# SinOncology/BreakID

Measured on AMD Instinct MI355X. Metric: M reads/s clustered+split-scanned, higher is better.
Workload: dtype int32/u8 (+f64 sd replay)

## Files before the change

breakid_amd/capi.py:

```python
from __future__ import annotations

import ctypes as C
import math
import os
import subprocess

import numpy as np

from . import abi

_HERE = os.path.dirname(os.path.abspath(__file__))
LIB_PATH = os.path.join(_HERE, "libbreakid_hip.so")
_LIB = None


class BreakIDError(RuntimeError):
    def __init__(self, code, msg):
        super().__init__("libbreakid_hip error %d: %s" % (code, msg))
        self.code = code


def build(verbose=False):
    cmd = ["make", "-C", os.path.join(_HERE, "csrc"), "-j8"]
    r = subprocess.run(cmd, capture_output=not verbose, text=True)
    if r.returncode != 0:
        raise RuntimeError("building libbreakid_hip.so failed:\n" + (r.stdout or "")[-4000:] + (r.stderr or "")[-4000:])


EXPORTS = ["bk_init", "bk_prepare_process", "bk_free", "bk_last_error", "bk_set_stream", "bk_sync", "bk_get_stream", "bk_upload_records", "bk_isize_stats",
           "bk_discordant_pairs", "bk_mask_and_cluster", "bk_split_evidence", "bk_cluster_summary",
           "bk_split_breakpoints", "bk_run", "bk_fetch", "bk_timing", "bk_timing_enable", "bk_timing_touched", "bk_group_stats", "bk_qname_hash", "bk_qname_check",
           "bk_bam_open", "bk_bam_header", "bk_bam_decode", "bk_bam_close", "bk_bam_decode_device", "bk_bam_decode_device_part", "bk_bam_decode_device_ctx", "bk_bam_dev_free", "bk_feed_release_caches", "bk_debug_bgzf_inflate", "bk_debug_std_sort", "bk_debug_ahc", "bk_debug_points", "bk_debug_cigar", "bk_debug_vote", "bk_debug_region", "bk_shard_begin", "bk_shard_get_stats", "bk_shard_set_stats",
           "bk_shard_sd_local", "bk_shard_sd_finish", "bk_shard_buffer", "bk_shard_set_buffer", "bk_shard_group_sizes",
           "bk_shard_own_groups", "bk_shard_route_candidates", "bk_shard_group_keys", "bk_shard_route_pairs", "bk_shard_group_pairs", "bk_shard_bp_cov", "bk_shard_bp_vote", "bk_shard_bp_vote_slice", "bk_shard_bp_set_voted", "bk_shard_bp_depth", "bk_shard_bp_finish"]


def lib():
    global _LIB
    if _LIB is None:
        if not os.path.exists(LIB_PATH):
            raise BreakIDError(abi.BK_ERR_NO_DEVICE, "libbreakid_hip.so is not built (run __graft_entry__.build()); "
                                                     "there is no CPU fallback")
        try:
            import torch
        except Exception:
            pass
        L = C.CDLL(LIB_PATH)
        vp, u64p, dp = C.c_void_p, C.POINTER(C.c_uint64), C.POINTER(C.c_double)
        L.bk_init.argtypes = [C.c_int, vp, C.POINTER(C.c_char_p), C.c_int, C.POINTER(vp)]
        L.bk_free.argtypes = [vp]
        L.bk_last_error.restype = C.c_char_p
        L.bk_last_error.argtypes = [vp]
        L.bk_set_stream.argtypes = [vp, vp]
        L.bk_sync.argtypes = [vp]
        L.bk_upload_records.argtypes = [vp, C.POINTER(abi.Soa), C.c_int]
        L.bk_isize_stats.argtypes = [vp, dp, dp]
        L.bk_discordant_pairs.argtypes = [vp, C.c_int, C.c_double, u64p, C.POINTER(C.c_uint32)]
        L.bk_mask_and_cluster.argtypes = [vp, C.c_double, C.c_int, u64p]
        L.bk_split_evidence.argtypes = [vp, u64p]
        L.bk_cluster_summary.argtypes = [vp, C.c_double, u64p]
        L.bk_split_breakpoints.argtypes = [vp, C.c_double, u64p]
        L.bk_run.argtypes = [vp, C.c_int, C.c_int, dp, u64p]
        L.bk_fetch.argtypes = [vp, C.c_int, C.POINTER(vp), u64p, C.POINTER(C.POINTER(C.c_uint64)), C.POINTER(C.c_uint32)]
        L.bk_timing.argtypes = [vp, C.POINTER(C.POINTER(C.c_char_p)), C.POINTER(C.POINTER(C.c_float)),
                                C.POINTER(C.POINTER(C.c_uint64)), C.POINTER(C.c_int)]
        L.bk_timing_enable.argtypes = [vp, C.c_int]
        L.bk_timing_touched.argtypes = [vp, C.POINTER(C.POINTER(C.c_uint64)), C.POINTER(C.c_int)]
        L.bk_debug_std_sort.argtypes = [vp, vp, vp, C.c_uint32, vp]
        L.bk_debug_ahc.argtypes = [vp, vp, vp, C.c_uint32, C.c_double, vp, vp, C.POINTER(C.c_uint32)]
        L.bk_debug_points.argtypes = [vp, C.c_int, vp, vp, C.c_uint32, C.c_double, vp, vp, C.POINTER(C.c_uint32)]
        L.bk_debug_cigar.argtypes = [vp, C.c_uint32, vp, vp, vp, vp, vp, vp, vp]
        L.bk_debug_vote.argtypes = [vp, vp, C.c_uint32, vp, C.c_uint32, C.c_int32, C.c_int32, vp]
        L.bk_debug_region.argtypes = [vp, C.c_int32, C.c_uint32, C.c_uint32, C.c_uint64, vp, C.c_uint32, C.POINTER(C.c_uint32), C.POINTER(C.c_uint32),
                                      C.POINTER(C.c_uint32)]
        L.bk_shard_begin.argtypes = [vp, C.c_uint64, C.c_int]
        L.bk_shard_get_stats.argtypes = [vp, C.POINTER(abi.ShardStats)]
        L.bk_shard_set_stats.argtypes = [vp, C.POINTER(abi.ShardStats)]
        L.bk_shard_sd_local.argtypes = [vp, u64p, C.POINTER(vp), u64p]
        L.bk_shard_sd_finish.argtypes = [vp, vp, C.c_uint64, C.c_uint64, dp, dp]
        L.bk_shard_buffer.argtypes = [vp, C.c_int, C.POINTER(vp), u64p, C.POINTER(C.c_uint32)]
        L.bk_shard_set_buffer.argtypes = [vp, C.c_int, vp, C.c_uint64]
        L.bk_shard_group_sizes.argtypes = [vp, C.POINTER(C.POINTER(C.c_uint64)), C.POINTER(C.c_uint32)]
        L.bk_shard_own_groups.argtypes = [vp, vp, C.c_uint32]
        L.bk_shard_route_candidates.argtypes = [vp, C.c_uint32, C.POINTER(vp), C.POINTER(C.POINTER(C.c_uint64))]
        L.bk_shard_group_keys.argtypes = [vp, C.POINTER(C.POINTER(C.c_uint32)), C.POINTER(C.c_uint32)]
        L.bk_shard_route_pairs.argtypes = [vp, vp, C.c_uint32, C.c_uint32, C.POINTER(vp), C.POINTER(C.POINTER(C.c_uint64))]
        L.bk_shard_group_pairs.argtypes = [vp, vp, C.c_uint64, vp, C.c_uint32]
        L.bk_shard_bp_cov.argtypes = [vp, C.c_double, C.POINTER(vp), u64p]
        L.bk_shard_bp_vote.argtypes = [vp, C.c_double, vp]
        L.bk_shard_bp_vote_slice.argtypes = [vp, C.c_double, vp, C.c_uint64, C.c_uint64, C.POINTER(vp), C.POINTER(vp)]
        L.bk_shard_bp_set_voted.argtypes = [vp, vp]
        L.bk_shard_bp_depth.argtypes = [vp, C.POINTER(vp), u64p]
        L.bk_shard_bp_finish.argtypes = [vp, vp]
        L.bk_qname_hash.restype = C.c_uint64
        L.bk_qname_hash.argtypes = [C.c_char_p, C.c_size_t]
        L.bk_qname_check.restype = C.c_uint32
        L.bk_qname_check.argtypes = [C.c_char_p, C.c_size_t]
        L.bk_bam_open.argtypes = [C.c_char_p, C.POINTER(vp), C.c_char_p, C.c_size_t]
        L.bk_bam_header.argtypes = [vp, C.POINTER(C.c_int), C.POINTER(C.POINTER(C.c_char_p)), C.POINTER(C.POINTER(C.c_uint32))]
        L.bk_bam_decode.argtypes = [vp, C.POINTER(abi.Soa), C.c_char_p, C.c_size_t]
        L.bk_bam_close.argtypes = [vp]
        L.bk_bam_decode_device.argtypes = [C.c_char_p, C.c_int, C.POINTER(vp), C.POINTER(abi.Soa), C.POINTER(C.c_int), C.POINTER(C.POINTER(C.c_char_p)),
                                           C.POINTER(C.POINTER(C.c_uint32)), C.c_char_p, C.c_size_t]
        L.bk_bam_decode_device_part.argtypes = [C.c_char_p, C.c_int, C.c_int, C.c_int, C.POINTER(vp), C.POINTER(abi.Soa), C.POINTER(C.c_int), C.POINTER(C.POINTER(C.c_char_p)),
                                           C.POINTER(C.POINTER(C.c_uint32)), C.c_char_p, C.c_size_t]
        L.bk_bam_dev_free.argtypes = [vp]
        L.bk_feed_release_caches.argtypes = []
        L.bk_feed_release_caches.restype = None
        L.bk_bam_decode_device_ctx.argtypes = [C.c_char_p, C.c_int, C.c_int, C.POINTER(vp), C.POINTER(vp), C.POINTER(C.c_int), C.POINTER(C.POINTER(C.c_char_p)),
                                               C.POINTER(C.POINTER(C.c_uint32)), C.c_char_p, C.c_size_t]
        L.bk_debug_bgzf_inflate.argtypes = [vp, C.c_uint64, vp, C.c_uint64, C.POINTER(C.c_uint64), C.POINTER(C.c_float), C.c_char_p, C.c_size_t]
        _LIB = L
    return _LIB


def w_from(mean, sd):
    times = 2
    return times * math.sqrt(times) * (mean + 3 * sd)


class Context:

    def __init__(self, contigs, device=0):
        self.L = lib()
        self.contigs = list(contigs)
        lens = np.asarray([l for _, l in contigs], dtype=np.uint32)
        names = (C.c_char_p * len(contigs))(*[n.encode() for n, _ in contigs])
        h = C.c_void_p()
        rc = self.L.bk_init(device, lens.ctypes.data, names, len(contigs), C.byref(h))
        if rc != 0:
            raise BreakIDError(rc, (self.L.bk_last_error(None) or b"").decode())
        self.h = h
        self._keep = None

    def close(self):
        if self.h:
            self.L.bk_free(self.h)
            self.h = None

    def __del__(self):
        try:
            self.close()
        except Exception:
            pass

    def _check(self, rc):
        if rc != 0:
            raise BreakIDError(rc, (self.L.bk_last_error(self.h) or b"").decode())

    def set_stream(self, hip_stream_handle):
        self._check(self.L.bk_set_stream(self.h, C.c_void_p(hip_stream_handle)))

    def sync(self):
        self._check(self.L.bk_sync(self.h))

    def upload(self, cols):
        qc = cols.get("qcheck")
        cols = {k: np.ascontiguousarray(cols[k], dtype=dt) for k, dt in abi.SOA_COLS}
        if qc is not None:
            cols["qcheck"] = np.ascontiguousarray(qc, dtype=np.uint32)
        for k in ("cigar", "aux"):
            if cols[k].size == 0:
                cols[k] = np.zeros(1, cols[k].dtype)
        soa = abi.soa_from_numpy(cols)
        self._keep = (cols, soa)
        self._check(self.L.bk_upload_records(self.h, C.byref(soa), abi.BK_MEM_HOST))

    def attach_device_table(self, table):
        self._keep = table
        self._check(self.L.bk_upload_records(self.h, C.byref(table.soa), abi.BK_MEM_DEVICE))

    def upload_soa(self, handle):
        self._keep = handle
        self._check(self.L.bk_upload_records(self.h, C.byref(handle.soa), abi.BK_MEM_HOST))

    def attach_device(self, ptrs, n, n_cigar_words, n_aux_bytes):
        s = abi.Soa()
        s.n = n
        for name, _ in abi.SOA_COLS:
            setattr(s, name, ptrs[name])
        if ptrs.get("qcheck"):
            s.qcheck = ptrs["qcheck"]
        if ptrs.get("side"):
            s.side = ptrs["side"]
        s.n_cigar_words = n_cigar_words
        s.n_aux_bytes = n_aux_bytes
        self._keep = (ptrs, s)
        self._check(self.L.bk_upload_records(self.h, C.byref(s), abi.BK_MEM_DEVICE))

    def isize_stats(self):
        m, s = C.c_double(), C.c_double()
        self._check(self.L.bk_isize_stats(self.h, C.byref(m), C.byref(s)))
        return m.value, s.value

    def discordant_pairs(self, qual, w):
        n, g = C.c_uint64(), C.c_uint32()
        self._check(self.L.bk_discordant_pairs(self.h, qual, w, C.byref(n), C.byref(g)))
        return n.value, g.value

    def mask_and_cluster(self, w, fast):
        n = C.c_uint64()
        self._check(self.L.bk_mask_and_cluster(self.h, w, int(fast), C.byref(n)))
        return n.value

    def split_evidence(self):
        n = C.c_uint64()
        self._check(self.L.bk_split_evidence(self.h, C.byref(n)))
        return n.value

    def cluster_summary(self, w):
        n = C.c_uint64()
        self._check(self.L.bk_cluster_summary(self.h, w, C.byref(n)))
        return n.value

    def split_breakpoints(self, w, count=True):
        n = C.c_uint64()
        self._check(self.L.bk_split_breakpoints(self.h, w, C.byref(n) if count else None))
        return n.value

    def run(self, qual=20, fast=True):
        w, n = C.c_double(), C.c_uint64()
        self._check(self.L.bk_run(self.h, qual, int(fast), C.byref(w), C.byref(n)))
        return w.value, n.value

    def fetch(self, stage):
        def fn(h, st, d, c, g, ng):
            return self.L.bk_fetch(h, st, d, c, g, ng)
        try:
            return abi.fetch_array(self.L, self.h, fn, stage)
        except RuntimeError:
            self._check(-1 if not self.L.bk_last_error(self.h) else abi.BK_ERR_ARG)
            raise

    def debug_std_sort(self, key, group_off):
        key = np.ascontiguousarray(key, np.uint32)
        group_off = np.ascontiguousarray(group_off, np.uint64)
        perm = np.zeros(len(key), np.uint32)
        self._check(self.L.bk_debug_std_sort(self.h, key.ctypes.data, group_off.ctypes.data, len(group_off) - 1, perm.ctypes.data))
        return perm

    def debug_ahc(self, x, y, w):
        x = np.ascontiguousarray(x, np.uint32)
        y = np.ascontiguousarray(y, np.uint32)
        n = len(x)
        idx = np.zeros(max(n, 1), np.uint32)
        cl = np.zeros(max(n, 1), np.int32)
        m = C.c_uint32()
        self._check(self.L.bk_debug_ahc(self.h, x.ctypes.data, y.ctypes.data, n, float(w), idx.ctypes.data, cl.ctypes.data, C.byref(m)))
        return idx[:m.value].copy(), cl[:m.value].copy()

    def debug_points(self, mode, x, y, w):
        x = np.ascontiguousarray(x, np.uint32)
        y = np.ascontiguousarray(y, np.uint32)
        n = len(x)
        idx = np.zeros(max(n, 1), np.uint32)
        cl = np.zeros(max(n, 1), np.int32)
        m = C.c_uint32()
        self._check(self.L.bk_debug_points(self.h, {"mask": 0, "iso": 1, "fast": 2}[mode], x.ctypes.data, y.ctypes.data, n, float(w), idx.ctypes.data,
                                           cl.ctypes.data, C.byref(m)))
        return idx[:m.value].copy(), cl[:m.value].copy()

    def debug_cigar(self, rows):
        kind = np.asarray([1 if r[0] == "b" else 0 for r in rows], np.uint8)
        c1 = bytearray()
        o1 = [0]
        for r in rows:
            while r[0] == "b" and len(c1) % 4:
                c1 += b"\0"
                o1[-1] = len(c1)
            c1 += np.asarray(r[1], np.uint32).tobytes() if r[0] == "b" else r[1].encode()
            o1.append(len(c1))
        c2 = bytearray()
        o2 = [0]
        for r in rows:
            c2 += r[2].encode()
            o2.append(len(c2))
        o1a, o2a = np.asarray(o1, np.uint32), np.asarray(o2, np.uint32)
        b1 = np.frombuffer(bytes(c1) + b"\0" * 16, np.uint8)
        b2 = np.frombuffer(bytes(c2) + b"\0" * 16, np.uint8)
        e = np.asarray([r[3] for r in rows], np.int32)
        out = np.zeros((len(rows), 6), np.int32)
        self._check(self.L.bk_debug_cigar(self.h, len(rows), kind.ctypes.data, o1a.ctypes.data, b1.ctypes.data, o2a.ctypes.data, b2.ctypes.data, e.ctypes.data,
                                          out.ctypes.data))
        return out

    def debug_vote(self, s1, s2, p1_tid, p2_tid):
        s1 = np.ascontiguousarray(s1, abi.SPLIT)
        s2 = np.ascontiguousarray(s2, abi.SPLIT)
        out = np.zeros(3, np.int32)
        self._check(self.L.bk_debug_vote(self.h, s1.ctypes.data, len(s1), s2.ctypes.data, len(s2), p1_tid, p2_tid, out.ctypes.data))
        return tuple(int(v) for v in out)

    def debug_region(self, tid, start, end, depth_pos, cap=4096):
        out = np.zeros(cap, abi.SPLIT)
        n, cov, depth = C.c_uint32(), C.c_uint32(), C.c_uint32()
        self._check(self.L.bk_debug_region(self.h, tid, start, end, depth_pos, out.ctypes.data, cap, C.byref(n), C.byref(cov), C.byref(depth)))
        return out[:min(n.value, cap)].copy(), n.value, cov.value, depth.value

    def timing_enable(self, on=True):
        self._check(self.L.bk_timing_enable(self.h, int(on)))

    def timing(self):
        names = C.POINTER(C.c_char_p)()
        ms = C.POINTER(C.c_float)()
        by = C.POINTER(C.c_uint64)()
        n = C.c_int()
        self._check(self.L.bk_timing(self.h, C.byref(names), C.byref(ms), C.byref(by), C.byref(n)))
        return [(names[i].decode(), float(ms[i]), int(by[i])) for i in range(n.value)]

    def timing_touched(self):
        t = C.POINTER(C.c_uint64)()
        n = C.c_int()
        self._check(self.L.bk_timing_touched(self.h, C.byref(t), C.byref(n)))
        return [int(t[i]) for i in range(n.value)]


class DeviceBamTable:

    def __init__(self, L, h, soa, contigs):
        self.L, self.h, self.soa, self.contigs = L, h, soa, contigs

    def close(self):
        if self.h:
            self.L.bk_bam_dev_free(self.h)
            self.h = None


def decode_bam_device(path, device=0):
    L = lib()
    h = C.c_void_p()
    err = C.create_string_buffer(512)
    s = abi.Soa()
    nt = C.c_int()
    names = C.POINTER(C.c_char_p)()
    lens = C.POINTER(C.c_uint32)()
    rc = L.bk_bam_decode_device(path.encode(), device, C.byref(h), C.byref(s), C.byref(nt), C.byref(names), C.byref(lens), err, 512)
    if rc != 0:
        raise BreakIDError(rc, err.value.decode())
    contigs = [(names[i].decode(), int(lens[i])) for i in range(nt.value)]
    return DeviceBamTable(L, h, s, contigs)


def decode_bam_device_part(path, part, parts, device=0):
    L = lib()
    h = C.c_void_p()
    err = C.create_string_buffer(512)
    s = abi.Soa()
    nt = C.c_int()
    names = C.POINTER(C.c_char_p)()
    lens = C.POINTER(C.c_uint32)()
    rc = L.bk_bam_decode_device_part(path.encode(), device, part, parts, C.byref(h), C.byref(s), C.byref(nt), C.byref(names), C.byref(lens), err, 512)
    if rc != 0:
        raise BreakIDError(rc, err.value.decode())
    contigs = [(names[i].decode(), int(lens[i])) for i in range(nt.value)]
    return DeviceBamTable(L, h, s, contigs)


def decode_bam_device_ctx(path, qual=20, device=0):
    L = lib()
    hb, hc = C.c_void_p(), C.c_void_p()
    err = C.create_string_buffer(512)
    nt = C.c_int()
    names = C.POINTER(C.c_char_p)()
    lens = C.POINTER(C.c_uint32)()
    rc = L.bk_bam_decode_device_ctx(path.encode(), device, qual, C.byref(hb), C.byref(hc), C.byref(nt), C.byref(names), C.byref(lens), err, 512)
    if rc != 0:
        raise BreakIDError(rc, err.value.decode())
    contigs = [(names[i].decode(), int(lens[i])) for i in range(nt.value)]
    ctx = Context.__new__(Context)
    ctx.L, ctx.contigs, ctx.h = L, contigs, hc
    table = DeviceBamTable(L, hb, None, contigs)
    ctx._keep = table
    return ctx, table


class BamTable:

    def __init__(self, L, h, soa):
        self.L, self.h, self.soa = L, h, soa
        n = soa.n
        self.nbytes = n * (4 * 5 + 2 + 1 + 8) + (n + 1) * 8 + soa.n_cigar_words * 4 + soa.n_aux_bytes

    def close(self):
        if self.h:
            self.L.bk_bam_close(self.h)
            self.h = None


def decode_bam(path, keep=False):
    L = lib()
    h = C.c_void_p()
    err = C.create_string_buffer(512)
    rc = L.bk_bam_open(path.encode(), C.byref(h), err, 512)
# ... 34 lines not shown
```

breakid_amd/csrc/api.hip:

```cpp
#include <algorithm>
#include <cmath>
#include <cstring>
#include <memory>
#include <numeric>
#include <thread>
#include <atomic>
#include <chrono>

#include "bk_common.h"
#include <dirent.h>
#include "prims.h"
#include "stream.h"
#include "join.h"
#include "cluster.h"
#include "bp.h"
#include "ahc.h"
#include "bgzf_gpu.h"

namespace
{
thread_local std::string g_init_error;

uint64_t fnv64(const std::string &s)
{
// ... 807 lines not shown
  if (want == 1 || want == 2) return want;
  return stage_queues() >= 2 * K ? 2 : 1;
}
static int lanes_wanted(bool svc)
{
  const char *env = getenv("BREAKID_GROUP_LANES");
  static const int want_svc = env ? atoi(env) : 12;
  if (svc) return want_svc < 1 ? 1 : (want_svc > 26 ? 26 : want_svc);
  static const int want = env ? atoi(env) : std::max(1, std::min(4, stage_queues() / lane_streams_each(std::min(4, stage_queues()))));
  return want < 1 ? 1 : (want > 26 ? 26 : want);
}
static bool lanes_apply(const bk_ctx *ctx, int fast)
{
  static const uint64_t min_pairs = getenv("BREAKID_LANES_MIN_PAIRS") ? strtoull(getenv("BREAKID_LANES_MIN_PAIRS"), nullptr, 10) : (1ull << 20);
  uint32_t large = 0;
  const uint64_t big = std::max<uint64_t>(2, min_pairs >> 6);
  for (uint32_t g = 0; g < ctx->jr.n_groups && g + 1 < ctx->gstart_host.size(); ++g) large += ctx->gstart_host[g + 1] - ctx->gstart_host[g] >= big ? 1u : 0u;
  const bool yes = lanes_wanted(lane_service(fast)) >= 2 && fast && ctx->jr.n_groups >= 4 && ctx->jr.n_pairs >= min_pairs && large >= 2;
  if (yes)
  {
    static bool told = false;
    const int K = lanes_wanted(lane_service(fast));
    if (!told && !lane_service(fast) && K * lane_streams_each(K) > stage_queues() && bk_debug("lanes"))
    {
      told = true;
      fprintf(stderr, "[breakid] GPU_MAX_HW_QUEUES=%d: the lanes of chromosome-pair groups (bk_mask_and_cluster) and their heap kernels will share hardware queues "
                        "(BREAKID_GROUP_LANES=1: one pass)\n", g_hw_queues_at_init);
    }
  }
  return yes;
}

struct LanePlan
{
  std::vector<int> lane_of;
};
static LanePlan plan_blind(const bk_ctx *ctx, int K)
{
  const uint32_t ng = ctx->jr.n_groups;
  std::vector<uint32_t> order(ng);
  std::iota(order.begin(), order.end(), 0u);
  auto size_of = [&](uint32_t g) { return ctx->gstart_host[g + 1] - ctx->gstart_host[g]; };
  std::stable_sort(order.begin(), order.end(), [&](uint32_t a, uint32_t b) { return size_of(a) > size_of(b); });
  constexpr double wexp = 2.0;
  LanePlan p;
  p.lane_of.assign(ng, 0);
  std::vector<double> load(K, 0.0);
  const bool owned_only = !ctx->own_groups.empty();
  if (owned_only && ctx->own_groups.size() != ng) throw bk_error(BK_ERR_ARG, "bk_shard_own_groups: group count changed");
  for (uint32_t i = 0; i < ng; ++i)
  {
    const uint32_t g = order[i];
    if (owned_only && !ctx->own_groups[g])
    {
      p.lane_of[g] = -1;
      continue;
    }
    int l = 0;
    for (int k = 1; k < K; ++k)
      if (load[k] < load[l]) l = k;
    load[l] += std::pow((double) size_of(g), wexp);
    p.lane_of[g] = l;
  }
  return p;
}
static LanePlan plan_observed(const std::vector<uint64_t> &sizes, const std::vector<uint32_t> &hx, const std::vector<uint32_t> &hy, int K, double x_sorts = 1.0)
{
  const uint32_t ng = (uint32_t) sizes.size();
  constexpr double per_pair = 0.001;
  auto heap_cost = [](uint32_t m) { return (double) m + (m > 40947u ? 1.0 * (double) (m - 40947u) : 0.0); };
  std::vector<uint32_t> order(ng);
  std::iota(order.begin(), order.end(), 0u);
  auto chain = [&](uint32_t g) { return heap_cost(hx[g]) + heap_cost(hy[g]); };
  std::stable_sort(order.begin(), order.end(), [&](uint32_t a, uint32_t b) {
    const double ca = chain(a), cb = chain(b);
    return ca != cb ? ca > cb : sizes[a] > sizes[b];
  });
  LanePlan p;
  p.lane_of.assign(ng, 0);
  std::vector<double> mx(K, 0.0), my(K, 0.0), pairs(K, 0.0);
  auto cost = [&](int l) { return x_sorts * mx[l] + my[l] + per_pair * pairs[l]; };
  for (uint32_t g : order)
  {
    const int l0 = 0;
    int best = l0;
    double best_cost = 0;
    for (int l = l0; l < K; ++l)
    {
      const double c = x_sorts * std::max(mx[l], heap_cost(hx[g])) + std::max(my[l], heap_cost(hy[g])) + per_pair * (pairs[l] + (double) sizes[g]);
      if (l == l0 || c < best_cost || (c == best_cost && cost(l) < cost(best)))
      {
        best = l;
        best_cost = c;
      }
    }
    mx[best] = std::max(mx[best], heap_cost(hx[g]));
    my[best] = std::max(my[best], heap_cost(hy[g]));
    pairs[best] += (double) sizes[g];
    p.lane_of[g] = best;
  }
  if (bk_debug("lanes"))
    for (int l = 0; l < K; ++l)
    {
      fprintf(stderr, "[lanes] lane %d: max heap x %.0f y %.0f, %.0f pairs, cost %.0f; heavy groups:", l, mx[l], my[l], pairs[l], cost(l));
      for (uint32_t g = 0; g < ng; ++g)
        if (p.lane_of[g] == l && (hx[g] || hy[g])) fprintf(stderr, " %u(%u,%u)", g, hx[g], hy[g]);
      fprintf(stderr, "\n");
    }
  return p;
}

static void group_lanes(bk_ctx *ctx, double w, int fast)
{
  const uint32_t ng = ctx->jr.n_groups;
  auto make_lanes = [&](int K, int S) {
    while ((int) ctx->lanes.size() < K - 1)
    {
      ctx->lanes.emplace_back(new bk_ctx::Lane());
      ctx->lanes.back()->cb.max_group_bound = ctx->cb.max_group_bound;
    }
    for (int k = 0; k < S - 1; ++k)
      if (!ctx->lanes[k]->st) HIP_CHECK(hipStreamCreateWithFlags(&ctx->lanes[k]->st, hipStreamNonBlocking));
  };
  bool use_svc = sort_service_on() && fast;
  if (use_svc && !lane_service(fast))
  {
    use_svc = false;
    tell_no_service();
    if (bk_debug("lanes")) fprintf(stderr, "[lanes] %d hardware queues, the sort service needs %d: not started\n", g_hw_queues_at_init, SVC_STAGE_QUEUES);
  }
  int K = lanes_wanted(use_svc);
  int S = use_svc ? std::max(1, std::min(LANE_STREAMS_MAX, K)) : K;
  make_lanes(K, S);
  std::vector<hipStream_t> stage_streams{ctx->st};
  for (int k = 0; k < S - 1; ++k) stage_streams.push_back(ctx->lanes[k]->st);
  SvcStage svc_stage(ctx, use_svc, ctx->jr.n_pairs + 2ull * ng + 4096, ctx->cb.max_group_bound, stage_streams);
  if (use_svc && !svc_stage.on)
  {
    use_svc = false;
    K = lanes_wanted(false);
    S = K;
    make_lanes(K, S);
  }
  struct ForkReset
  {
    bk_ctx *c;
    ~ForkReset() { c->cb.se.fork_heaps = true; }
  } fork_reset{ctx};
  {
    const bool fork = use_svc || lane_streams_each(K) == 2;
    ctx->cb.se.fork_heaps = fork;
    for (int k = 0; k < K - 1; ++k) ctx->lanes[k]->cb.se.fork_heaps = fork;
    if (!use_svc && bk_debug("lanes")) fprintf(stderr, "[lanes] launch path: %d lanes, %d stream%s each, %d hardware queues\n", K, fork ? 2 : 1, fork ? "s" : "", g_hw_queues_at_init);
  }
  const bool adapt = !use_svc;
  auto lane_cb = [&](int l) -> ClusterBufs & { return l == 0 ? ctx->cb : ctx->lanes[l - 1]->cb; };
  auto lane_st = [&](int l) { const int k = l % S; return k == 0 ? ctx->st : ctx->lanes[k - 1]->st; };
  auto lane_list = [&](int l) -> PairList & { return l == 0 ? ctx->listA : ctx->lanes[l - 1]->list; };
  auto lane_iso = [&](int l) -> PairList & { return l == 0 ? ctx->isoA : ctx->lanes[l - 1]->iso; };
  auto lane_cl = [&](int l) -> DevBuf & { return l == 0 ? ctx->d_clusterA : ctx->lanes[l - 1]->d_cluster; };
  uint32_t *drop_base = nullptr;
  auto lane_drop = [&](int l) { return drop_base + (size_t) l * ((size_t) ng + 1); };
  std::vector<std::vector<uint8_t>> keep(K, std::vector<uint8_t>(ng, 0));
  auto upload_plan = [&](const LanePlan &p) {
    for (int l = 0; l < K; ++l)
      for (uint32_t g = 0; g < ng; ++g) keep[l][g] = p.lane_of[g] == l ? 1 : 0;
    std::vector<uint32_t> drop((size_t) K * ((size_t) ng + 1), 0u);
    for (int l = 0; l < K; ++l)
      for (uint32_t g = 0; g < ng; ++g) drop[(size_t) l * ((size_t) ng + 1) + g] = p.lane_of[g] == l ? 0u : 1u;
    drop_base = ctx->d_dropA.as<uint32_t>(drop.size() + 1);
    HIP_CHECK(hipMemcpyAsync(drop_base, drop.data(), drop.size() * 4, hipMemcpyHostToDevice, ctx->st));
    HIP_CHECK(hipStreamSynchronize(ctx->st));
  };
  auto in_lanes = [&](auto body) {
    std::vector<std::string> err(K);
    std::vector<int> code(K, BK_OK);
    static const bool dbg_lanes = bk_debug("lanes");
    const auto t_start = std::chrono::steady_clock::now();
    auto guarded_body = [&](int l) {
      try
      {
        body(l);
        HIP_CHECK(hipStreamSynchronize(lane_st(l)));
        if (dbg_lanes)
          fprintf(stderr, "[lanes] lane %d done after %.2f ms\n", l, std::chrono::duration<double, std::milli>(std::chrono::steady_clock::now() - t_start).count());
      }
      catch (const bk_error &e)
      {
        code[l] = e.code;
        err[l] = e.msg;
      }
    };
    std::vector<std::thread> th;
    for (int l = 1; l < K; ++l)
      th.emplace_back([&, l] {
        (void) hipSetDevice(ctx->device);
        guarded_body(l);
      });
    guarded_body(0);
    for (std::thread &t : th) t.join();
    for (int l = 0; l < K; ++l)
      if (code[l] != BK_OK) throw bk_error(code[l], err[l]);
  };
  auto merge_all = [&](auto list_of, auto cl_of, PairList &out, DevBuf *cl_out, PairList *, DevBuf *) {
    std::vector<const PairList *> ls(K);
    std::vector<const uint32_t *> cs(K);
    for (int l = 0; l < K; ++l)
    {
      ls[l] = &list_of(l);
      cs[l] = cl_of(l);
    }
    merge_lists_many(ls.data(), cl_out ? cs.data() : nullptr, K, out, cl_out, ctx->st);
  };
  const bk_pair *pairs = ctx->jr.pairs;
  static const bool dbg_phases = bk_debug("lanes");
  const auto tp0 = std::chrono::steady_clock::now();
  auto phase = [&](const char *what) {
    if (dbg_phases) fprintf(stderr, "[lanes] %s at %.2f ms\n", what, std::chrono::duration<double, std::milli>(std::chrono::steady_clock::now() - tp0).count());
  };
  upload_plan(plan_blind(ctx, K));
  phase("plan uploaded");
  phase("service started");
  if (!adapt)
  {
    in_lanes([&](int l) { run_lane(pairs, ctx->jr.gof, ctx->jr.gstart, ng, ctx->jr.n_pairs, w, fast, lane_drop(l), lane_list(l), lane_iso(l), lane_cl(l), lane_cb(l), ctx->ab, lane_st(l), ctx->gstart_host.data(), keep[l].data()); });
  }
  else
  {
    constexpr bool split_early = false;
    in_lanes([&](int l) {
      ClusterBufs &cb = lane_cb(l);
      cb.heavy_x.assign(ng, 0u);
      cb.heavy_y.assign(ng, 0u);
      cb.observe = true;
      cb.se.heavy_all = false;
      remove_isolated_begin(pairs, ctx->jr.gof, ctx->jr.gstart, ng, ctx->jr.n_pairs, w, lane_list(l), cb, lane_st(l), lane_drop(l), ctx->gstart_host.data(), keep[l].data());
      if (!split_early)
      {
        cb.heavy_x.assign(ng, 0u);
        remove_isolated_end(pairs, lane_list(l), cb, lane_st(l));
      }
      cb.observe = false;
    });
    PairList &mid = ctx->lane_mid;
    PairList *acc = ctx->lane_acc;
    DevBuf *cacc = ctx->lane_cacc;
    merge_all([&](int l) -> const PairList & { return lane_list(l); }, [&](int) -> const uint32_t * { return nullptr; }, mid, nullptr, acc, cacc);
    std::vector<uint64_t> goff_h((size_t) ng + 1);
    HIP_CHECK(hipMemcpyAsync(goff_h.data(), mid.goff.get<uint64_t>(), ((size_t) ng + 1) * 8, hipMemcpyDeviceToHost, ctx->st));
    HIP_CHECK(hipStreamSynchronize(ctx->st));
    std::vector<uint64_t> sizes(ng);
    std::vector<uint32_t> hx(ng, 0u), hy(ng, 0u);
    for (uint32_t g = 0; g < ng; ++g) sizes[g] = goff_h[g + 1] - goff_h[g];
    for (int l = 0; l < K; ++l)
      for (uint32_t g = 0; g < ng; ++g)
      {
        hx[g] = std::max(hx[g], lane_cb(l).heavy_x[g]);
        hy[g] = std::max(hy[g], lane_cb(l).heavy_y[g]);
      }
    upload_plan(plan_observed(sizes, hx, hy, K, split_early ? 2.0 : 1.0));
    in_lanes([&](int l) {
      PairList &L = lane_list(l), &iso = lane_iso(l);
      hipStream_t st = lane_st(l);
      list_subset_ranges(mid, goff_h.data(), keep[l].data(), L, st);
      if (split_early) remove_isolated_end(pairs, L, lane_cb(l), st);
      iso.n = L.n;
      iso.ng = L.ng;
      uint32_t *ii = iso.idx.as<uint32_t>(L.n + 1), *ig = iso.gof.as<uint32_t>(L.n + 1);
      uint64_t *io = iso.goff.as<uint64_t>((uint64_t) L.ng + 1);
      if (L.n) HIP_CHECK(hipMemcpyAsync(ii, L.idx.get<uint32_t>(), L.n * 4, hipMemcpyDeviceToDevice, st));
      if (L.n) HIP_CHECK(hipMemcpyAsync(ig, L.gof.get<uint32_t>(), L.n * 4, hipMemcpyDeviceToDevice, st));
      HIP_CHECK(hipMemcpyAsync(io, L.goff.get<uint64_t>(), ((uint64_t) L.ng + 1) * 8, hipMemcpyDeviceToDevice, st));
      if (fast)
        fast_cluster_all(pairs, L, w, lane_cl(l), lane_cb(l), st);
      else
        ahc_cluster_all(pairs, L, w, lane_cl(l), ctx->ab, lane_cb(l), st);
    });
  }
  phase("lanes done");
  svc_stage.finish();
  phase("service stopped");
  if (use_svc && bk_debug("lanes")) fprintf(stderr, "[svc] tasks: %u wide, %u narrow\n", ctx->svc.stats[0], ctx->svc.stats[1]);
  PairList &iso_m = ctx->lane_iso_m;
  PairList *iacc = ctx->lane_acc, *lacc = ctx->lane_acc + 2;
  DevBuf *icacc = ctx->lane_cacc, *lcacc = ctx->lane_cacc + 2;
  merge_all([&](int l) -> const PairList & { return lane_iso(l); }, [&](int) -> const uint32_t * { return nullptr; }, iso_m, nullptr, iacc, icacc);
  merge_all([&](int l) -> const PairList & { return lane_list(l); }, [&](int l) -> const uint32_t * { return lane_cl(l).get<uint32_t>(); }, ctx->list, &ctx->d_cluster, lacc, lcacc);
  HIP_CHECK(hipStreamSynchronize(ctx->st));
  phase("lists merged");
  ctx->iso_n = iso_m.n;
  std::swap(ctx->iso_idx, iso_m.idx);
  std::swap(ctx->iso_goff, iso_m.goff);
}

int bk_mask_and_cluster(bk_ctx *ctx, double w, int fast, uint64_t *n_clustered)
{
  return guarded(ctx, [&] {
    {
      uint64_t mg = 0;
      for (uint32_t g = 0; g < ctx->jr.n_groups && g + 1 < ctx->gstart_host.size(); ++g) mg = std::max<uint64_t>(mg, ctx->gstart_host[g + 1] - ctx->gstart_host[g]);
      ctx->cb.max_group_bound = mg;
      for (auto &l : ctx->lanes) l->cb.max_group_bound = mg;
    }
    if (lanes_apply(ctx, fast))
    {
      {
// ... 294 lines not shown
    if (n_groups) *n_groups = ctx->jr.n_groups;
  });
}

int bk_shard_own_groups(bk_ctx *ctx, const uint8_t *own, uint32_t n_groups)
{
  return guarded(ctx, [&] {
    if (n_groups != ctx->jr.n_groups) throw bk_error(BK_ERR_ARG, "bk_shard_own_groups: wrong group count");
    ctx->own_groups.assign(own, own + n_groups);
  });
}

int bk_shard_route_candidates(bk_ctx *ctx, uint32_t world, void **dev, const uint64_t **counts)
{
  return guarded(ctx, [&] {
    if (!ctx->stream_done || ctx->ext_cand) throw bk_error(BK_ERR_ARG, "bk_shard_route_candidates: needs this shard's own candidates (after bk_shard_begin)");
    if (!world || world > 4096 || !dev || !counts) throw bk_error(BK_ERR_ARG, "bk_shard_route_candidates: bad arguments");
    *dev = route_candidates(ctx->d_cand.get<Cand>(), ctx->hc.n_cand, world, ctx->jb, ctx->st, ctx->route_counts);
    *counts = ctx->route_counts.data();
  });
}

int bk_shard_group_keys(bk_ctx *ctx, const uint32_t **keys, uint32_t *n_groups)
{
  return guarded(ctx, [&] {
    if (keys) *keys = ctx->gkey_host.data();
    if (n_groups) *n_groups = ctx->jr.n_groups;
  });
}

int bk_shard_route_pairs(bk_ctx *ctx, const uint32_t *dest_of_group, uint32_t n_groups, uint32_t world, void **dev, const uint64_t **counts)
{
  return guarded(ctx, [&] {
    if (n_groups != ctx->jr.n_groups || !world || !dev || !counts || (n_groups && !dest_of_group)) throw bk_error(BK_ERR_ARG, "bk_shard_route_pairs: bad arguments");
    ctx->route_counts.assign(world, 0);
    for (uint32_t g = 0; g < n_groups; ++g)
    {
      if (dest_of_group[g] >= world) throw bk_error(BK_ERR_ARG, "bk_shard_route_pairs: destination out of range");
      ctx->route_counts[dest_of_group[g]] += ctx->gstart_host[g + 1] - ctx->gstart_host[g];
    }
    std::vector<uint64_t> base(world, 0), off(n_groups, 0);
    for (uint32_t d = 1; d < world; ++d) base[d] = base[d - 1] + ctx->route_counts[d - 1];
    for (uint32_t g = 0; g < n_groups; ++g)
    {
      off[g] = base[dest_of_group[g]];
      base[dest_of_group[g]] += ctx->gstart_host[g + 1] - ctx->gstart_host[g];
    }
    *dev = route_pairs(ctx->jr, off, ctx->jb, ctx->st);
    *counts = ctx->route_counts.data();
  });
}

int bk_shard_group_pairs(bk_ctx *ctx, const void *pairs_dev, uint64_t n, const uint32_t *all_keys, uint32_t n_all_keys)
{
  return guarded(ctx, [&] {
    if ((n && !pairs_dev) || (n_all_keys && !all_keys)) throw bk_error(BK_ERR_ARG, "bk_shard_group_pairs: null input");
    {
      Scope s(ctx, "group_pairs");
      ctx->jb2.rec_bits = -1;
      group_pairs((const bk_pair *) pairs_dev, n, ctx->nt, ctx->jb2, ctx->st, ctx->jr);
    }
    std::vector<uint32_t> keys(all_keys, all_keys + n_all_keys);
    finish_groups(ctx, &keys);
    ctx->own_groups.clear();
    ctx->clustered = false;
  });
}

int bk_shard_bp_cov(bk_ctx *ctx, double w, void **cov_dev, uint64_t *n)
{
  return guarded(ctx, [&] {
    uint32_t *cov = bp_cov_partial(rec_view(ctx), ctx->clusters_ptr(), ctx->n_clusters, w, (int) ctx->hc.max_span, ctx->bb, ctx->st);
    HIP_CHECK(hipStreamSynchronize(ctx->st));
    if (cov_dev) *cov_dev = cov;
    if (n) *n = 2 * ctx->n_clusters;
  });
}

int bk_shard_bp_vote(bk_ctx *ctx, double w, const void *cov_total_dev)
{
  return guarded(ctx, [&] {
    ensure_splits_sorted(ctx);
    bp_vote(ctx->d_split.get<bk_split>(), ctx->hc.n_split, ctx->clusters_ptr(), ctx->n_clusters, w, (int) ctx->hc.max_span, (const uint32_t *) cov_total_dev,
            ctx->d_hdr.get<int32_t>(), ctx->bb, ctx->st);
    HIP_CHECK(hipStreamSynchronize(ctx->st));
  });
}

int bk_shard_bp_vote_slice(bk_ctx *ctx, double w, const void *cov_total_dev, uint64_t lo, uint64_t hi, void **clusters_dev, void **voted_dev)
{
  return guarded(ctx, [&] {
    if (lo > hi || hi > ctx->n_clusters || !clusters_dev || !voted_dev) throw bk_error(BK_ERR_ARG, "bk_shard_bp_vote_slice: bad range");
    ensure_splits_sorted(ctx);
    bp_vote(ctx->d_split.get<bk_split>(), ctx->hc.n_split, ctx->clusters_ptr() + lo, hi - lo, w, (int) ctx->hc.max_span,
            cov_total_dev ? (const uint32_t *) cov_total_dev + 2 * lo : nullptr, ctx->d_hdr.get<int32_t>(), ctx->bb, ctx->st);
    HIP_CHECK(hipStreamSynchronize(ctx->st));
    *clusters_dev = ctx->clusters_ptr() + lo;
    *voted_dev = ctx->bb.voted.p;
  });
}

int bk_shard_bp_set_voted(bk_ctx *ctx, const void *voted_all_dev)
{
  return guarded(ctx, [&] {
    uint32_t *v = ctx->bb.voted.as<uint32_t>(ctx->n_clusters + 1);
    if (ctx->n_clusters && voted_all_dev != v)
      HIP_CHECK(hipMemcpyAsync(v, voted_all_dev, ctx->n_clusters * 4, hipMemcpyDeviceToDevice, ctx->st));
    HIP_CHECK(hipStreamSynchronize(ctx->st));
  });
}

int bk_shard_bp_depth(bk_ctx *ctx, void **depth_dev, uint64_t *n)
{
  return guarded(ctx, [&] {
    uint32_t *d = bp_depth_partial(rec_view(ctx), ctx->clusters_ptr(), ctx->n_clusters, (int) ctx->hc.max_span, ctx->bb, ctx->st);
    HIP_CHECK(hipStreamSynchronize(ctx->st));
    if (depth_dev) *depth_dev = d;
    if (n) *n = 2 * ctx->n_clusters;
  });
}

int bk_shard_bp_finish(bk_ctx *ctx, const void *depth_total_dev)
{
  return guarded(ctx, [&] {
    bp_finish(ctx->clusters_ptr(), ctx->n_clusters, (const uint32_t *) depth_total_dev, ctx->bb, ctx->st);
    HIP_CHECK(hipStreamSynchronize(ctx->st));
  });
}

int bk_debug_std_sort(bk_ctx *ctx, const uint32_t *key, const uint64_t *group_off, uint32_t n_groups, uint32_t *perm_out)
{
  return guarded(ctx, [&] {
    if (!key || !group_off || !perm_out) throw bk_error(BK_ERR_ARG, "bk_debug_std_sort: null argument");
    const uint64_t n = group_off[n_groups];
    DevBuf dk, dp, dgof, dgoff;
    std::vector<uint32_t> gof(n), iota(n);
    for (uint32_t g = 0; g < n_groups; ++g)
      for (uint64_t p = group_off[g]; p < group_off[g + 1]; ++p) gof[p] = g;
    std::iota(iota.begin(), iota.end(), 0u);
    HIP_CHECK(hipMemcpy(dk.as<uint32_t>(n + 1), key, n * 4, hipMemcpyHostToDevice));
    HIP_CHECK(hipMemcpy(dp.as<uint32_t>(n + 1), iota.data(), n * 4, hipMemcpyHostToDevice));
    HIP_CHECK(hipMemcpy(dgof.as<uint32_t>(n + 1), gof.data(), n * 4, hipMemcpyHostToDevice));
    HIP_CHECK(hipMemcpy(dgoff.as<uint64_t>((uint64_t) n_groups + 1), group_off, ((uint64_t) n_groups + 1) * 8, hipMemcpyHostToDevice));
    uint64_t max_group = 0;
    for (uint32_t g = 0; g < n_groups; ++g) max_group = std::max<uint64_t>(max_group, group_off[g + 1] - group_off[g]);
    SvcStage svc_stage(ctx, true, n + 2ull * n_groups + 4096, max_group, {ctx->st});
    std_sort_groups(dk.get<uint32_t>(), dp.get<uint32_t>(), dgof.get<uint32_t>(), dgoff.get<uint64_t>(), n_groups, n, ctx->cb.se, ctx->st);
    svc_stage.finish();
    HIP_CHECK(hipMemcpyAsync(perm_out, dp.get<uint32_t>(), n * 4, hipMemcpyDeviceToHost, ctx->st));
    HIP_CHECK(hipStreamSynchronize(ctx->st));
  });
}

int bk_debug_ahc(bk_ctx *ctx, const uint32_t *x, const uint32_t *y, uint32_t n, double w, uint32_t *idx_out, int32_t *cluster_out, uint32_t *n_out)
{
  return guarded(ctx, [&] {
    if (!x || !y || !idx_out || !cluster_out || !n_out) throw bk_error(BK_ERR_ARG, "bk_debug_ahc: null argument");
    std::vector<bk_pair> hp(n);
    for (uint32_t i = 0; i < n; ++i)
    {
      memset(&hp[i], 0, sizeof(bk_pair));
      hp[i].x = x[i];
      hp[i].y = y[i];
    }
    DevBuf dp, dcl;
    PairList L;
    L.n = n;
    L.ng = 1;
    std::vector<uint32_t> iota(n), gof(n, 0);
    std::iota(iota.begin(), iota.end(), 0u);
    uint64_t goff[2] = {0, n};
    HIP_CHECK(hipMemcpy(dp.as<bk_pair>(n + 1), hp.data(), n * sizeof(bk_pair), hipMemcpyHostToDevice));
    HIP_CHECK(hipMemcpy(L.idx.as<uint32_t>(n + 1), iota.data(), n * 4, hipMemcpyHostToDevice));
    HIP_CHECK(hipMemcpy(L.gof.as<uint32_t>(n + 1), gof.data(), n * 4, hipMemcpyHostToDevice));
    HIP_CHECK(hipMemcpy(L.goff.as<uint64_t>(2), goff, 16, hipMemcpyHostToDevice));
    ahc_cluster_all(dp.get<bk_pair>(), L, w, dcl, ctx->ab, ctx->cb, ctx->st);
    *n_out = (uint32_t) L.n;
    if (L.n)
    {
      HIP_CHECK(hipMemcpyAsync(idx_out, L.idx.get<uint32_t>(), L.n * 4, hipMemcpyDeviceToHost, ctx->st));
      HIP_CHECK(hipMemcpyAsync(cluster_out, dcl.get<uint32_t>(), L.n * 4, hipMemcpyDeviceToHost, ctx->st));
    }
    HIP_CHECK(hipStreamSynchronize(ctx->st));
  });
}

}

namespace
{
struct FeedLink
{
  int device = 0, mapq_min = 20;
  bk_ctx *ctx = nullptr;
  int rc = BK_OK;
  std::string err;
  uint64_t done = 0;
  bool prepared = false, overflow = false;
  hipEvent_t t0 = nullptr, t1 = nullptr;
  template <class F> void guard(F &&f)
  {
    if (rc != BK_OK) return;
    try
    {
      f();
    }
    catch (const bk_error &e)
    {
      rc = e.code;
      err = e.msg;
    }
  }
};
void link_header(void *u, int nt, const char *const *names, const uint32_t *lens)
{
  FeedLink *L = (FeedLink *) u;
  if (L->ctx || L->rc != BK_OK) return;
  L->rc = bk_init(L->device, lens, names, nt, &L->ctx);
  if (L->rc != BK_OK) L->err = bk_last_error(nullptr);
}
void link_reset(void *u)
{
  FeedLink *L = (FeedLink *) u;
  L->guard([&] {
    if (L->ctx) HIP_CHECK(hipStreamSynchronize(L->ctx->st));
    L->done = 0;
    L->prepared = false;
    L->overflow = false;
  });
}
void link_before_move(void *u)
{
  FeedLink *L = (FeedLink *) u;
  L->guard([&] {
    if (L->ctx) HIP_CHECK(hipStreamSynchronize(L->ctx->st));
  });
}
void link_chunk(void *u, const bk_soa *cols, uint64_t n_ready, uint64_t n_est, hipEvent_t ready)
{
  FeedLink *L = (FeedLink *) u;
  L->guard([&] {
    bk_ctx *c = L->ctx;
    if (!c || n_ready < (uint64_t) STREAM_V + 1) return;
    c->rec = *cols;
    c->have_records = true;
    c->mapq_min = L->mapq_min;
    if (!L->prepared)
    {
      stream_prepare(c, n_est + n_est / 4);
      L->prepared = true;
    }
    const uint64_t lim = (n_ready - 1) / STREAM_V * STREAM_V;
    if (lim <= L->done) return;
    HIP_CHECK(hipStreamWaitEvent(c->st, ready, 0));
    StreamArgs a = stream_args(c, lim);
    a.q_begin = L->done / STREAM_V;
    launch_stream(a, c->st);
    L->done = lim;
  });
}
}


extern "C" {

int bk_bam_decode_device_ctx(const char *path, int device, int mapq_min, bk_bam_dev **bam_out, bk_ctx **ctx_out, int *n_targets, const char *const **names,
                             const uint32_t **lens, char *err, size_t errlen)
{
  auto fail = [&](int code, const std::string &m) {
    if (err && errlen) snprintf(err, errlen, "%s", m.c_str());
    return code;
  };
  if (!path || !bam_out || !ctx_out) return fail(BK_ERR_ARG, "bk_bam_decode_device_ctx: null argument");
  *bam_out = nullptr;
  *ctx_out = nullptr;
  FeedLink L;
  L.device = device;
  L.mapq_min = mapq_min;
  FeedConsumer fc;
  fc.user = &L;
  fc.on_header = link_header;
  fc.on_chunk = link_chunk;
  fc.before_move = link_before_move;
  fc.on_reset = link_reset;
  bk_soa cols;
  bk_bam_dev *bam = nullptr;
  int rc = bam_decode_device_impl(path, device, &bam, &cols, n_targets, names, lens, err, errlen, &fc);
  if (rc == BK_OK && L.rc != BK_OK) rc = fail(L.rc, L.err);
  if (rc == BK_OK && !L.ctx) rc = fail(BK_ERR_IO, "bk_bam_decode_device_ctx: no header");
  if (rc != BK_OK)
  {
    if (L.ctx) bk_free(L.ctx);
    if (bam) bk_bam_dev_free(bam);
    return rc;
  }
  bk_ctx *c = L.ctx;
  rc = guarded(c, [&] {
    const uint64_t done = L.prepared ? L.done : 0;
    c->stream_done = c->stats_done = c->clustered = false;
    c->rec = cols;
    c->have_records = true;
    c->mapq_min = mapq_min;
    c->rec_base = 0;
    bool ok = false;
    if (L.prepared)
    {
// ... 243 lines not shown
```

breakid_amd/csrc/sortemu.h:

```cpp
#pragma once
#include "bk_common.h"
#include "prims.h"
#include <vector>
#include <atomic>

struct SortService
{
  DevBuf ctl, slots[2], seq[2], jobs, dbg, pos[2];
  uint32_t pos_cap[2] = {0, 0};
  uint32_t cap[2] = {0, 0};
  hipStream_t st[2] = {nullptr, nullptr}, quit_stream = nullptr, st_copy = nullptr;
  uint32_t *quit_host = nullptr;
  uint32_t *quit_dev = nullptr;
  uint32_t cap32 = 0;
  uint32_t quit_word = 0, starts = 0;
  size_t wide_lds = 0;
  bool running = false;
  std::atomic<uint32_t> next_slot{0};
  uint32_t stats[8] = {};
  void start(uint64_t n_bound, uint64_t max_group, hipStream_t after);
  bool narrow_running(double seconds) const;
  void stop();
  uint32_t new_slot() { return next_slot.fetch_add(1u); }
  ~SortService();
  SortService() = default;
  SortService(const SortService &) = delete;
  SortService &operator=(const SortService &) = delete;
};

struct SortEmuBufs
{
  SortService *svc = nullptr;
  uint32_t svc_slot = 0xFFFFFFFFu, svc_epoch = 0;
  DevBuf cnt, err, segs_a, segs_b, posL, posR, scan_tmp, heap_list, heap_scratch, scratch32, scratch32b, fin_list, lv_tile, lv_segbase, lv_tileseg, lv_bar, chk_key0, chk_cnt, chk_bad, rk_a, rk_b, heap_tickets;
  prims::RadixBufs radix;
  std::vector<uint32_t> *heavy = nullptr;
  bool heavy_all = false;
  bool fork_heaps = true;
  static constexpr int N_AUX = 5;
  hipStream_t aux[N_AUX] = {};
  hipEvent_t fork = nullptr, join[N_AUX] = {};
  SortEmuBufs() = default;
  SortEmuBufs(const SortEmuBufs &) = delete;
  SortEmuBufs &operator=(const SortEmuBufs &) = delete;
  ~SortEmuBufs()
  {
    for (int i = 0; i < N_AUX; ++i)
    {
      if (aux[i]) (void) hipStreamDestroy(aux[i]);
      if (join[i]) (void) hipEventDestroy(join[i]);
    }
    if (fork) (void) hipEventDestroy(fork);
  }
};

void std_sort_groups(uint32_t *key, uint32_t *idx, const uint32_t *gof, const uint64_t *goff, uint32_t ng, uint64_t n, SortEmuBufs &b, hipStream_t st);
```

breakid_amd/csrc/sortemu.hip:

```cpp
#include "bk_common.h"
#include "prims.h"
#include "sortemu.h"
#include <vector>
#include <mutex>
#include <algorithm>
#include <cstdio>
#include <chrono>
#include <thread>
#include <cstdlib>
#include <ctime>

namespace
{
inline double now_ms()
{
  timespec ts;
  clock_gettime(CLOCK_MONOTONIC, &ts);
  return ts.tv_sec * 1e3 + ts.tv_nsec * 1e-6;
}
typedef __attribute__((address_space(1))) uint32_t gu32_t;
__device__ __forceinline__ void st_through(uint32_t *p, uint32_t v) { __hip_atomic_store((gu32_t *) p, v, __ATOMIC_RELAXED, __HIP_MEMORY_SCOPE_AGENT); }
struct Seg
{
  uint32_t first, last;
// ... 899 lines not shown
  const uint32_t budget = __builtin_amdgcn_readfirstlane(64u * (m - cap) + 4096u);
  const uint32_t mm = __builtin_amdgcn_readfirstlane(m), cc = __builtin_amdgcn_readfirstlane(cap);
  const unsigned long long o = (unsigned long long) out, pp = (unsigned long long) ovf;
  const uint32_t olo = __builtin_amdgcn_readfirstlane((uint32_t) o), ohi = __builtin_amdgcn_readfirstlane((uint32_t) (o >> 32));
  const uint32_t plo = __builtin_amdgcn_readfirstlane((uint32_t) pp), phi = __builtin_amdgcn_readfirstlane((uint32_t) (pp >> 32));
  const uint32_t base = __builtin_amdgcn_readfirstlane((uint32_t) (unsigned long long) slot1);
  uint32_t left;
  asm volatile(BK_HEAP32H_ASM
               : [left] "=s"(left)
               : [olo] "s"(olo), [ohi] "s"(ohi), [plo] "s"(plo), [phi] "s"(phi), [base] "s"(base), [m] "s"(mm), [cap] "s"(cc), [budget] "s"(budget)
               : BK_HEAP_CLOBBERS, "v68", "v69", "v70", "v71", "s64", "s65", "s66", "s67", "s68", "s69", "s70");
  asm volatile("s_waitcnt vmcnt(0) lgkmcnt(0)" ::: "memory");
  if (lane == 0)
  {
    atomicAdd(&g_heap_iters[0], (unsigned long long) (budget - left) + (m - cap));
    atomicAdd(&g_heap_iters[1], (unsigned long long) (m - cap));
  }
}

constexpr uint32_t HEAP_SMALL = 1024;
constexpr uint32_t HEAP_LARGE = 20000;
constexpr size_t HEAP_BIG_LDS = 163800;
constexpr uint32_t HEAP_LARGE32 = HEAP_BIG_LDS / 4 - 3;
constexpr uint32_t HEAP_RANKED_MIN = 4096;
constexpr uint32_t HEAP_RANKED_MAX = 65534;

constexpr uint32_t HEAP_BIG_THREADS = 1024;
constexpr uint32_t RK_UNROLL = 4;
__device__ void wg_ranked_entries(const uint32_t *gk, const uint32_t m, unsigned long long *A, unsigned long long *B, uint32_t *out, uint32_t *lds, uint32_t *wcnt, const uint32_t NT)
{
  const uint32_t tid = threadIdx.x, lane = tid & 63, w = tid >> 6, NW = NT >> 6;
  for (uint32_t i = tid; i < m; i += NT) A[i] = ((unsigned long long) gk[i] << 16) | i;
  const uint32_t rows = (m + 63) / 64, rpw = (rows + NW - 1) / NW;
  const uint32_t r0 = min(rows, w * rpw), r1 = min(rows, r0 + rpw);
  unsigned long long *src = A, *dst = B;
  __syncthreads();
  for (int pass = 0; pass < 4; ++pass)
  {
    const int sh = 16 + 8 * pass;
    uint32_t *hist = lds + w * 256;
    for (uint32_t d = lane; d < 256; d += 64) hist[d] = 0;
    for (uint32_t r = r0; r < r1; r += RK_UNROLL)
    {
      unsigned long long e[RK_UNROLL];
#pragma unroll
      for (uint32_t u = 0; u < RK_UNROLL; ++u)
      {
        const uint32_t i = (r + u) * 64 + lane;
        e[u] = (r + u < r1 && i < m) ? src[i] : ~0ull;
      }
#pragma unroll
      for (uint32_t u = 0; u < RK_UNROLL; ++u)
        if (e[u] != ~0ull) atomicAdd(&hist[(uint32_t) (e[u] >> sh) & 255u], 1u);
    }
    __syncthreads();
    if (tid < 256)
    {
      uint32_t tot = 0;
      for (uint32_t k = 0; k < NW; ++k) tot += lds[k * 256 + tid];
      uint32_t inc = tot;
      for (int d = 1; d < 64; d <<= 1)
      {
        const uint32_t o = __shfl_up(inc, d, 64);
        if ((int) lane >= d) inc += o;
      }
      if (lane == 63) wcnt[w] = inc;
      lds[NW * 256 + tid] = inc - tot;
    }
    __syncthreads();
    if (tid < 256)
    {
      uint32_t base = lds[NW * 256 + tid];
      for (uint32_t k = 0; k < w; ++k) base += wcnt[k];
      for (uint32_t k = 0; k < NW; ++k)
      {
        const uint32_t c = lds[k * 256 + tid];
        lds[k * 256 + tid] = base;
        base += c;
      }
    }
    __syncthreads();
    for (uint32_t r = r0; r < r1; r += RK_UNROLL)
    {
      unsigned long long e[RK_UNROLL];
#pragma unroll
      for (uint32_t u = 0; u < RK_UNROLL; ++u)
      {
        const uint32_t i = (r + u) * 64 + lane;
        e[u] = (r + u < r1 && i < m) ? src[i] : ~0ull;
      }
#pragma unroll
      for (uint32_t u = 0; u < RK_UNROLL; ++u)
      {
        const bool valid = e[u] != ~0ull;
        const uint32_t d = (uint32_t) (e[u] >> sh) & 255u;
        unsigned long long peers = __ballot(valid);
#pragma unroll
        for (int bit = 0; bit < 8; ++bit)
        {
          const bool mine = (d >> bit) & 1u;
          const unsigned long long bal = __ballot(mine);
          peers &= mine ? bal : ~bal;
        }
        const uint32_t before = __builtin_amdgcn_mbcnt_hi((uint32_t) (peers >> 32), __builtin_amdgcn_mbcnt_lo((uint32_t) peers, 0u));
        const uint32_t base = valid ? hist[d] : 0u;
        if (valid) dst[base + before] = e[u];
        if (valid && before == 0) hist[d] = base + (uint32_t) __popcll(peers);
      }
    }
    __syncthreads();
    unsigned long long *t = src;
    src = dst;
    dst = t;
  }
  uint32_t changes = 0;
  for (uint32_t r = r0; r < r1; ++r)
  {
    const uint32_t i = r * 64 + lane;
    const bool ch = i < m && i > 0 && (src[i] >> 16) != (src[i - 1] >> 16);
    changes += (uint32_t) __popcll(__ballot(ch));
  }
  if (lane == 0) wcnt[w] = changes;
  __syncthreads();
  uint32_t run = 0;
  for (uint32_t k = 0; k < w; ++k) run += wcnt[k];
  __syncthreads();
  for (uint32_t r = r0; r < r1; r += RK_UNROLL)
  {
    unsigned long long e[RK_UNROLL], ep[RK_UNROLL];
#pragma unroll
    for (uint32_t u = 0; u < RK_UNROLL; ++u)
    {
      const uint32_t i = (r + u) * 64 + lane;
      const bool in = r + u < r1 && i < m;
      e[u] = in ? src[i] : ~0ull;
      ep[u] = in && i > 0 ? src[i - 1] : ~0ull;
    }
#pragma unroll
    for (uint32_t u = 0; u < RK_UNROLL; ++u)
    {
      const bool valid = e[u] != ~0ull;
      const bool ch = valid && ep[u] != ~0ull && (e[u] >> 16) != (ep[u] >> 16);
      const unsigned long long mk = __ballot(ch);
      const uint32_t upto = __builtin_amdgcn_mbcnt_hi((uint32_t) (mk >> 32), __builtin_amdgcn_mbcnt_lo((uint32_t) mk, 0u)) + (ch ? 1u : 0u);
      if (valid)
      {
        const uint32_t pos = (uint32_t) e[u] & 0xFFFFu;
        out[pos] = ((run + upto + 1u) << 16) | pos;
      }
      run += (uint32_t) __popcll(mk);
    }
  }
}
__device__ __forceinline__ void heap_small_body(const uint32_t first, const uint32_t last, uint32_t *key, uint32_t *idx, hent *buf, const uint32_t NT)
{
  const uint32_t m = last - first;
  uint32_t *gk = key + first, *gx = idx + first;
  for (uint32_t i = threadIdx.x; i < m; i += NT) buf[i] = ((hent) gk[i] << 32) | gx[i];
  __syncthreads();
  if (threadIdx.x < 64)
  {
    LdsMem mem{buf};
    make_heap_wave(mem, m);
    sort_heap_asm<false>(buf, m, 1);
  }
  __syncthreads();
  for (uint32_t i = threadIdx.x; i < m; i += NT)
  {
    const hent e = buf[i];
    st_through(gk + i, hkey(e));
    st_through(gx + i, (uint32_t) e);
  }
}
__device__ __forceinline__ void heap_big_body(const uint32_t first, const uint32_t last, uint32_t *key, uint32_t *idx, hent *scratch, uint32_t *scratch32, uint32_t *scratch32b,
                                              unsigned long long *rka, unsigned long long *rkb, hent *dyn, const uint32_t cap32, const uint32_t NT)
{
  const uint32_t m = last - first;
  uint32_t *gk = key + first, *gx = idx + first;
  hent *buf = scratch + first;
  const bool w0 = threadIdx.x < 64;
  for (uint32_t i = threadIdx.x; i < m; i += NT) buf[i] = ((hent) gk[i] << 32) | gx[i];
  __syncthreads();
  if (m <= HEAP_RANKED_MAX)
  {
    const unsigned long long tp0 = wall_clock64();
    uint32_t *l32 = reinterpret_cast<uint32_t *>(dyn);
    uint32_t *g32 = scratch32 + first;
    const bool fits = m <= cap32;
    unsigned long long tp1, tp2, tp3;
    if (fits)
    {
      wg_ranked_entries(gk, m, rka + first, rkb + first, l32 + 1, l32, l32 + (NT / 64 + 1) * 256, NT);
      __syncthreads();
      if (threadIdx.x < 3) l32[threadIdx.x == 0 ? 0 : m + threadIdx.x] = 0;
      __syncthreads();
      tp1 = wall_clock64();
      {
        LdsMemT<E32> mem{l32 + 1};
        make_heap_block(mem, m, NT);
      }
      tp2 = tp3 = wall_clock64();
      if (w0) sort_heap_lds_q(l32 + 1, m, g32);
    }
    else
    {
      wg_ranked_entries(gk, m, rka + first, rkb + first, g32, l32, l32 + (NT / 64 + 1) * 256, NT);
      asm volatile("s_waitcnt vmcnt(0)" ::: "memory");
      __syncthreads();
      tp1 = wall_clock64();
      {
        GlbMemT<E32> gmem{g32};
        make_heap_block(gmem, m, NT);
      }
      tp2 = wall_clock64();
      if (m < 2 * (cap32 + 1))
      {
        uint32_t *ovf = scratch32b + first;
        __syncthreads();
        for (uint32_t i = threadIdx.x; i < m; i += NT)
        {
          const uint32_t e = g32[i];
          if (i < cap32) l32[1 + i] = e; else ovf[1 + i] = e;
        }
        if (threadIdx.x < 3) l32[threadIdx.x == 0 ? 0 : cap32 + threadIdx.x] = 0;
        if (threadIdx.x < 2) ovf[m + 1 + threadIdx.x] = 0;
        asm volatile("s_waitcnt vmcnt(0)" ::: "memory");
        __syncthreads();
        if (w0) sort_heap_hybrid(l32 + 1, m, cap32, ovf, g32);
        tp3 = wall_clock64();
      }
      else
      {
        if (w0)
        {
          sort_heap_asm32<true>(g32, m, cap32);
          asm volatile("s_waitcnt vmcnt(0)" ::: "memory");
        }
        tp3 = wall_clock64();
        __syncthreads();
        for (uint32_t i = threadIdx.x; i < cap32; i += NT) l32[1 + i] = g32[i];
        if (threadIdx.x < 3) l32[threadIdx.x == 0 ? 0 : cap32 + threadIdx.x] = 0;
      }
      __syncthreads();
      if (w0) sort_heap_lds_q(l32 + 1, cap32, g32);
    }
    __syncthreads();
    if (threadIdx.x == 0) g32[0] = l32[1];
    asm volatile("s_waitcnt vmcnt(0) lgkmcnt(0)" ::: "memory");
    __syncthreads();
    const unsigned long long tp4 = wall_clock64();
    if (threadIdx.x == 0 && m > 36000)
    {
      g_heap_phase[0] = m;
      g_heap_phase[1] = tp1 - tp0;
      g_heap_phase[2] = tp2 - tp1;
      g_heap_phase[3] = tp3 - tp2;
      g_heap_phase[4] = tp4 - tp3;
    }
    for (uint32_t i = threadIdx.x; i < m; i += NT)
    {
      const hent e = buf[g32[i] & 0xFFFFu];
      st_through(gk + i, hkey(e));
      st_through(gx + i, (uint32_t) e);
    }
    return;
  }
  if (w0)
  {
    GlbMem gmem{buf};
    asm volatile("s_waitcnt vmcnt(0)" ::: "memory");
    make_heap_wave(gmem, m);
    sort_heap_asm<true>(buf, m, HEAP_LARGE);
    asm volatile("s_waitcnt vmcnt(0)" ::: "memory");
  }
  __syncthreads();
  for (uint32_t i = threadIdx.x; i < HEAP_LARGE; i += NT) dyn[i] = buf[i];
  __syncthreads();
  if (w0) sort_heap_asm<false>(dyn, HEAP_LARGE, 1);
  __syncthreads();
  for (uint32_t i = threadIdx.x; i < HEAP_LARGE; i += NT) buf[i] = dyn[i];
  asm volatile("s_waitcnt vmcnt(0)" ::: "memory");
  __syncthreads();
  for (uint32_t i = threadIdx.x; i < m; i += NT)
  {
    const hent e = buf[i];
    st_through(gk + i, hkey(e));
    st_through(gx + i, (uint32_t) e);
  }
}
template <int CLS> __global__ __launch_bounds__(CLS == 2 ? HEAP_BIG_THREADS : 64) void k_se_heapsort(const HeapSeg *__restrict__ hs, uint32_t nh, uint32_t *key, uint32_t *idx, hent *scratch, uint32_t lo, uint32_t hi,
                                                                                                    uint32_t *scratch32, uint32_t *scratch32b, unsigned long long *rka, unsigned long long *rkb)
{
  extern __shared__ __attribute__((aligned(16))) hent dyn[];
  __shared__ hent stat[CLS == 0 ? HEAP_SMALL + HEAP_PAD : 1];
  const uint32_t s = blockIdx.x;
  if (s >= nh) return;
  const HeapSeg sg = hs[s];
  const uint32_t m = sg.last - sg.first;
  if (m <= lo || m > hi) return;
  if (CLS == 2)
    heap_big_body(sg.first, sg.last, key, idx, scratch, scratch32, scratch32b, rka, rkb, dyn, HEAP_LARGE32, HEAP_BIG_THREADS);
  else
    heap_small_body(sg.first, sg.last, key, idx, CLS == 0 ? stat : dyn, 64);
}
__device__ __forceinline__ void heap_wave_body(const uint32_t first, const uint32_t last, uint32_t *key, uint32_t *idx, hent *buf)
{
  const uint32_t m = last - first, lane = threadIdx.x & 63;
  uint32_t *gk = key + first, *gx = idx + first;
  for (uint32_t i = lane; i < m; i += 64) buf[i] = ((hent) gk[i] << 32) | gx[i];
  asm volatile("s_waitcnt vmcnt(0) lgkmcnt(0)" ::: "memory");
  __builtin_amdgcn_wave_barrier();
  LdsMem mem{buf};
  make_heap_wave(mem, m);
  sort_heap_asm<false>(buf, m, 1);
  asm volatile("s_waitcnt lgkmcnt(0)" ::: "memory");
  __builtin_amdgcn_wave_barrier();
  for (uint32_t i = lane; i < m; i += 64)
  {
    const hent e = buf[i];
    st_through(gk + i, hkey(e));
// ... 1103 lines not shown
      int have = 0;
      for (int k = 0; k < n_wide; ++k) have += started[k] != 0u;
      if (have == n_wide) break;
      if (std::chrono::duration<double>(std::chrono::steady_clock::now() - t0).count() > 0.25) break;
    }
  }
  hipLaunchKernelGGL(k_sort_service<false>, dim3(n_narrow), dim3(256), SVC_NARROW_LDS, st[1], P);
  HIP_CHECK(hipGetLastError());
}
bool SortService::narrow_running(double seconds) const
{
  const auto t0 = std::chrono::steady_clock::now();
  volatile const uint32_t *flag = quit_host + SVC_H_NARROW;
  while (*flag == 0u)
    if (std::chrono::duration<double>(std::chrono::steady_clock::now() - t0).count() > seconds) return false;
  return true;
}
void SortService::stop()
{
  if (!running) return;
  running = false;
  __atomic_store_n(quit_host, quit_word, __ATOMIC_SEQ_CST);
  (void) hipMemcpyAsync(ctl.get<uint32_t>() + 192, quit_host, 4, hipMemcpyHostToDevice, st_copy);
  hipLaunchKernelGGL(k_svc_quit, dim3(1), dim3(1), 0, quit_stream, ctl.get<uint32_t>() + 192, quit_word);
  HIP_CHECK(hipStreamSynchronize(st[0]));
  HIP_CHECK(hipStreamSynchronize(st[1]));
  uint32_t h[40] = {};
  HIP_CHECK(hipMemcpy(h, ctl.get<uint32_t>() + 128, sizeof h, hipMemcpyDeviceToHost));
  for (int k = 0; k < 8; ++k) stats[k] = h[32 + k];
  DeferredFrees::end();
  if (bk_debug("svc"))
  {
    uint32_t c[128] = {};
    SvcJob j0 = {};
    HIP_CHECK(hipMemcpy(c, ctl.get<uint32_t>(), sizeof c, hipMemcpyDeviceToHost));
    HIP_CHECK(hipMemcpy(&j0, jobs.get<SvcJob>(), sizeof j0, hipMemcpyDeviceToHost));
    if (dbg.p)
    {
      std::vector<uint32_t> d(12 * 8192 + 48);
      HIP_CHECK(hipMemcpy(d.data(), dbg.p, d.size() * 4, hipMemcpyDeviceToHost));
      {
        const uint32_t *ph = d.data() + 12 * 8192 + 32;
        const double lv = ph[7] ? (double) ph[7] : 1.0;
        fprintf(stderr, "[svc]   wide partition nodes: %u levels; per level: count pass %.2f us, place pass %.2f us, swaps + drain %.2f us, cut, release, pushes and the next pivot %.2f us\n", ph[7], ph[0] * 1e-2 / lv,
                ph[1] * 1e-2 / lv, ph[2] * 1e-2 / lv, ph[3] * 1e-2 / lv);
      }
      for (int kind = 0; kind < 2; ++kind)
      {
        fprintf(stderr, "[svc]   %s tasks by size (2^k ..):", kind ? "narrow heap" : "finisher");
        for (int k = 4; k < 13; ++k) fprintf(stderr, " %d:%u", k, d[12 * 8192 + 16 * kind + k]);
        fprintf(stderr, "\n");
      }
      for (int kind = 0; kind < 2; ++kind)
      {
        const uint32_t nw = kind == 0 ? stats[2] : stats[3];
        double sum[8] = {};
        uint32_t longest = 0;
        for (uint32_t w = 0; w < nw && w < 4096; ++w)
        {
          const uint32_t *a = d.data() + 4 * 8192 + 8 * (w + 4096 * kind);
          for (int k = 0; k < 7; ++k) sum[k] += a[k];
          longest = std::max(longest, a[7]);
        }
        fprintf(stderr, "[svc]   %s workgroups (%u): waiting %.2f ms; partition nodes %.0f in %.2f ms, finisher %.0f in %.2f ms, heaps %.0f in %.2f ms (sums over the workgroups); longest task %.3f ms\n", kind ? "narrow" : "wide", nw,
                sum[0] * 1e-5, sum[4], sum[1] * 1e-5, sum[5], sum[2] * 1e-5, sum[6], sum[3] * 1e-5, longest * 1e-5);
        std::map<uint32_t, int> hist;
        const uint32_t n = kind == 0 ? stats[2] : stats[3];
        for (uint32_t w = 0; w < n && w < 4096; ++w) hist[d[4 * (w + 4096 * kind)]]++;
        fprintf(stderr, "[svc]   %s workgroups by last state (1 polling, 5 took a task, 9 left):", kind ? "narrow" : "wide");
        for (auto &kv : hist) fprintf(stderr, " %u:%d", kv.first, kv.second);
        fprintf(stderr, "; first ones (state, polls, time of the last poll in 10 ns, how it left 6 error 7 quit 8 timeout):");
        for (uint32_t w = 0; w < 6 && w < n; ++w) fprintf(stderr, " [%u %u %u %u]", d[4 * (w + 4096 * kind)], d[4 * (w + 4096 * kind) + 1], d[4 * (w + 4096 * kind) + 2], d[4 * (w + 4096 * kind) + 3]);
        fprintf(stderr, "\n");
      }
    }
    uint32_t sq[4] = {};
    HIP_CHECK(hipMemcpy(sq, seq[1].get<uint32_t>(), sizeof sq, hipMemcpyDeviceToHost));
    fprintf(stderr, "[svc] tasks %u wide / %u narrow; workgroups started %u / %u, left on their own %u / %u, odd quit words read %u; error %u; wide queue head %u tail %u, narrow queue head %u tail %u (seq %u %u %u %u); job 0: remaining %u done %u heaps %u (longest %u)\n",
            stats[0], stats[1], stats[2], stats[3], stats[4], stats[5], stats[6], h[0], c[0], c[32], c[64], c[96], sq[0], sq[1], sq[2], sq[3], j0.remaining, j0.done, j0.n_heap, j0.max_heap);
  }
  if (h[0]) throw bk_error(h[0] & 2u ? BK_ERR_LIMIT : BK_ERR_HIP, "sort service: task error " + std::to_string(h[0]) + " (2 = ring overflow, 4 = a job timed out, 8 = a cut outside its segment, 16 = a task in the wrong queue, 32 = a node beyond the position lists, 64 = the finisher); first failing task: code " + std::to_string(h[8]) + ", " + std::to_string(h[9]) + " " + std::to_string(h[10]) + " " + std::to_string(h[11]));
}
SortService::~SortService()
{
  if (running)
  {
    running = false;
    if (quit_host && st_copy)
    {
      __atomic_store_n(quit_host, quit_word, __ATOMIC_SEQ_CST);
      (void) hipMemcpyAsync(ctl.get<uint32_t>() + 192, quit_host, 4, hipMemcpyHostToDevice, st_copy);
    }
    if (quit_stream) hipLaunchKernelGGL(k_svc_quit, dim3(1), dim3(1), 0, quit_stream, ctl.get<uint32_t>() + 192, quit_word);
    for (int k = 0; k < 2; ++k)
      if (st[k]) (void) hipStreamSynchronize(st[k]);
    DeferredFrees::end();
  }
  for (int k = 0; k < 2; ++k)
    if (st[k]) (void) hipStreamDestroy(st[k]);
  if (st_copy) (void) hipStreamDestroy(st_copy);
  if (quit_host) (void) hipHostFree(quit_host);
}

static void window_sorts(uint32_t *key, uint32_t *idx, const uint32_t *gof, uint32_t n, hipStream_t st);

static void std_sort_groups_svc(uint32_t *key, uint32_t *idx, const uint32_t *gof, const uint64_t *goff, uint32_t ng, uint32_t n, SortEmuBufs &b, hipStream_t st)
{
  SortService &S = *b.svc;
  if (b.svc_slot == 0xFFFFFFFFu)
  {
    b.svc_slot = S.new_slot();
    if (b.svc_slot >= SVC_MAX_JOBS) throw bk_error(BK_ERR_LIMIT, "sort service: more than 64 callers");
  }
  SvcJob d = {};
  d.key = key;
  d.idx = idx;
  d.posL = b.posL.as<uint32_t>((uint64_t) n + 2);
  d.posR = b.posR.as<uint32_t>((uint64_t) n + 2);
  d.hscratch = b.heap_scratch.as<hent>((uint64_t) n + HEAP_PAD);
  d.scratch32 = b.scratch32.as<uint32_t>((uint64_t) n + HEAP_PAD);
  d.scratch32b = b.scratch32b.as<uint32_t>((uint64_t) n + HEAP_PAD);
  d.rka = b.rk_a.as<unsigned long long>((uint64_t) n + HEAP_PAD);
  d.rkb = b.rk_b.as<unsigned long long>((uint64_t) n + HEAP_PAD);
  d.epoch = (b.svc_epoch++ % 0xFFFFFu) + 1u;
  const SvcParams P = svc_params(S);
  hipLaunchKernelGGL(k_svc_submit, dim3(1), dim3(256), 0, st, P, d, b.svc_slot, goff, ng);
  HIP_CHECK(hipGetLastError());
  {
    volatile const uint32_t *done = S.quit_host + SVC_H_DONE + b.svc_slot, *err = S.quit_host + SVC_H_ERROR;
    const auto t0 = std::chrono::steady_clock::now();
    for (uint32_t spins = 0; *done != d.epoch; ++spins)
    {
      if (*err != 0u)
        throw bk_error(BK_ERR_HIP, "sort service: a task failed (error " + std::to_string(*err) + "; first failing task: code " + std::to_string(err[1]) + ", " + std::to_string(err[2]) + " " + std::to_string(err[3]) + " " + std::to_string(err[4]) + ")");
      if ((spins & 1023u) == 1023u)
      {
        if (std::chrono::duration<double>(std::chrono::steady_clock::now() - t0).count() > 20.0) throw bk_error(BK_ERR_HIP, "sort service: a job did not finish");
        std::this_thread::yield();
      }
      else
        __builtin_ia32_pause();
    }
  }
  if (bk_debug("svc"))
  {
    SvcJob j;
    HIP_CHECK(hipMemcpy(&j, S.jobs.get<SvcJob>() + b.svc_slot, sizeof j, hipMemcpyDeviceToHost));
    fprintf(stderr, "[svc] slot %u sort %u: %u elements in %u groups; partitions and finisher done after %.3f ms, job after %.3f ms; %u elements in heaps, the longest %u, the heap that ended last %u elements in %.3f ms\n", b.svc_slot,
            b.svc_epoch, n, ng, (double) (j.t_parts - j.t_submit) * 1e-5, (double) (j.t_done - j.t_submit) * 1e-5, j.n_heap, j.max_heap, (uint32_t) j.last_heap, (double) (j.last_heap >> 32) * 1e-5);
  }
  window_sorts(key, idx, gof, n, st);
}

void std_sort_groups(uint32_t *key, uint32_t *idx, const uint32_t *gof, const uint64_t *goff, uint32_t ng, uint64_t n64, SortEmuBufs &b, hipStream_t st)
{
  if (n64 == 0 || ng == 0) return;
  if (n64 > 0x7FFFFFF0ull) throw bk_error(BK_ERR_LIMIT, "std_sort_groups: more than 2^31 pairs");
  {
    static std::mutex flag_m;
    static bool flag_set[64] = {};
    int dev = 0;
    HIP_CHECK(hipGetDevice(&dev));
    std::lock_guard<std::mutex> l(flag_m);
    if (dev >= 0 && dev < 64 && !flag_set[dev])
    {
      const int nq = getenv("BK_HEAP_NO_Q") != nullptr;
      HIP_CHECK(hipMemcpyToSymbol(HIP_SYMBOL(g_heap_no_q), &nq, sizeof nq));
      const int nhy = nq;
      HIP_CHECK(hipMemcpyToSymbol(HIP_SYMBOL(g_heap_no_hybrid), &nhy, sizeof nhy));
      flag_set[dev] = true;
    }
  }
  const uint32_t n = (uint32_t) n64;
  if (b.svc && b.svc->running)
  {
    std_sort_groups_svc(key, idx, gof, goff, ng, n, b, st);
    return;
  }
  static const bool chk = bk_debug("sortcheck");
  DevBuf &chk_key0 = b.chk_key0;
  uint32_t *key0 = nullptr;
  if (chk)
  {
    key0 = chk_key0.as<uint32_t>(n);
    std::vector<uint32_t> hk(n), hx(n), k0(n);
    HIP_CHECK(hipStreamSynchronize(st));
    HIP_CHECK(hipMemcpy(hk.data(), key, (size_t) n * 4, hipMemcpyDeviceToHost));
    HIP_CHECK(hipMemcpy(hx.data(), idx, (size_t) n * 4, hipMemcpyDeviceToHost));
    for (uint32_t i = 0; i < n; ++i)
      if (hx[i] < n) k0[hx[i]] = hk[i];
    HIP_CHECK(hipMemcpy(key0, k0.data(), (size_t) n * 4, hipMemcpyHostToDevice));
    sort_check("at entry", key, idx, key0, n, goff, ng, st, b);
  }
  unsigned long long *cnt = b.cnt.as<unsigned long long>((uint64_t) (n / 8 + ng) + 32);
  if (const char *dump = getenv("BK_DEBUG_SORT_DUMP"))
  {
    static int call = 0;
    if (call < 5)
    {
      std::vector<uint64_t> go((size_t) ng + 1);
      std::vector<uint32_t> kk(n);
      HIP_CHECK(hipStreamSynchronize(st));
      HIP_CHECK(hipMemcpy(go.data(), goff, ((size_t) ng + 1) * 8, hipMemcpyDeviceToHost));
      HIP_CHECK(hipMemcpy(kk.data(), key, (size_t) n * 4, hipMemcpyDeviceToHost));
      char name[512];
      snprintf(name, sizeof name, "%s.%d.keys.u32", dump, call);
      if (FILE *f = fopen(name, "wb"))
      {
        fwrite(kk.data(), 4, kk.size(), f);
        fclose(f);
      }
      snprintf(name, sizeof name, "%s.%d.goff.u64", dump, call);
      if (FILE *f = fopen(name, "wb"))
      {
        fwrite(go.data(), 8, go.size(), f);
        fclose(f);
      }
    }
    ++call;
  }
  const uint32_t fin_cap = (uint32_t) ((uint64_t) n / 16 + ng + 16);
  FinSeg *fin_list = b.fin_list.as<FinSeg>(fin_cap);
  size_t max_segs = (size_t) n / 8 + ng + 16;
  Seg *segs = b.segs_a.as<Seg>(max_segs), *segs2 = b.segs_b.as<Seg>(max_segs);
  uint2 *heap_list = b.heap_list.as<uint2>(max_segs);
  uint32_t *state = b.err.as<uint32_t>(ST_WORDS);
  uint32_t *err = state + ST_ERR, *fin = state + ST_FIN, *lvl = state + ST_LVL;
  hipLaunchKernelGGL(k_se_reset, dim3(1), dim3(64), 0, st, state, fin_cap, (uint32_t) (max_segs - 1));
  hipLaunchKernelGGL(k_se_init, dim3(cdiv(ng, 256)), dim3(256), 0, st, goff, ng, cnt, fin_list, fin, lvl + 2);
  prims::exclusive_scan<unsigned long long>(cnt, cnt, ng, b.scan_tmp, st);
  unsigned long long tot = 0;
  uint32_t max_live = 0xFFFFFFFFu;
  HIP_CHECK(hipMemcpyAsync(&tot, cnt + ng, 8, hipMemcpyDeviceToHost, st));
  HIP_CHECK(hipMemcpyAsync(&max_live, lvl + 2, 4, hipMemcpyDeviceToHost, st));
  HIP_CHECK(hipStreamSynchronize(st));
  uint32_t ns = (uint32_t) tot, na = (uint32_t) (tot >> 32);
  if (ns)
  {
    hipLaunchKernelGGL(k_se_init_write, dim3(cdiv(ng, 256)), dim3(256), 0, st, goff, ng, cnt, segs, b.lv_tileseg.as<uint32_t>((uint64_t) n / LV_TILE + 2), lvl);
    unsigned long long *tile_cnt = b.lv_tile.as<unsigned long long>((uint64_t) n / LV_TILE + 2);
    unsigned long long *segbase = b.lv_segbase.as<unsigned long long>(max_segs + 1);
    uint32_t *tile_seg = b.lv_tileseg.as<uint32_t>((uint64_t) n / LV_TILE + 2);
    uint32_t *posL = b.posL.as<uint32_t>((uint64_t) n + 2), *posR = b.posR.as<uint32_t>((uint64_t) n + 2);
    int level = 0;
    static const bool dbg_levels = bk_debug("sort");
    double t_loop0 = 0;
    if (dbg_levels)
    {
      HIP_CHECK(hipStreamSynchronize(st));
      t_loop0 = now_ms();
    }
    bool pivoted = false;
    while (ns)
    {
      if (ns > max_segs) throw bk_error(BK_ERR_LIMIT, "std_sort_groups: segment list overflow");
      static const bool no_tail = getenv("BK_SORT_NO_TAIL") != nullptr;
      constexpr uint32_t tail_max = 1u << 19;
      constexpr int tail_level = 4;
      if (!no_tail && level >= tail_level && max_live <= tail_max)
      {
        if (!pivoted) hipLaunchKernelGGL(k_se_pivot, dim3(cdiv(ns, 256)), dim3(256), 0, st, segs, ns, key, idx, err, heap_list);
        int rounds = 1;
        for (uint64_t sz = max_live; sz / 2 > FIN_MAX; sz /= 2) ++rounds;
        uint32_t *rc = b.lv_bar.as<uint32_t>((uint64_t) rounds + 2);
        HIP_CHECK(hipMemsetAsync(rc, 0, ((size_t) rounds + 2) * 4, st));
        HIP_CHECK(hipMemcpyAsync(rc, &ns, 4, hipMemcpyHostToDevice, st));
        const uint32_t cap = (uint32_t) std::min<uint64_t>(max_segs, (uint64_t) na / FIN_MAX + 1);
        for (int r = 0; r < rounds; ++r)
        {
          const uint64_t bound = r < 1 ? std::min<uint64_t>(cap, ns) : cap;
          hipLaunchKernelGGL(k_se_tail_round, dim3((unsigned) std::max<uint64_t>(1, bound)), dim3(TL_THREADS), 0, st, (const Seg *) segs, (const uint32_t *) (rc + r), segs2, rc + r + 1, cap, key,
                             idx, posL, posR, fin_list, fin, err, heap_list, 1);
          std::swap(segs, segs2);
        }
        if (dbg_levels)
        {
          HIP_CHECK(hipStreamSynchronize(st));
          fprintf(stderr, "[sortemu]   levels %d.. by one workgroup per live segment in %d rounds: %u segments, %u live elements, largest %u, %.3f ms so far\n", level, rounds, ns, na, max_live, now_ms() - t_loop0);
        }
        break;
      }
      int batch = 0;
      constexpr int max_batch = 6;
      {
        if (ns <= CHILD_FUSED && na / FIN_MAX <= CHILD_FUSED)
          batch = max_batch;
        else
          for (uint32_t cap = ns; cap <= CHILD_FUSED && batch < max_batch; cap *= 2) ++batch;
      }
      if (batch == 0)
      {
        if (!pivoted) hipLaunchKernelGGL(k_se_pivot, dim3(cdiv(ns, 256)), dim3(256), 0, st, segs, ns, key, idx, err, heap_list);
        pivoted = false;
        {
          const unsigned nbt = cdiv(na, LV_TILE);
          hipLaunchKernelGGL(k_lv_count, dim3(nbt), dim3(256), 0, st, segs, ns, key, na, tile_cnt, (const uint32_t *) nullptr, (const uint32_t *) tile_seg);
          hipLaunchKernelGGL(k_lv_sums, dim3(1), dim3(LV_SUM_THREADS), 0, st, tile_cnt, ns, na, segbase, (const uint32_t *) nullptr);
          hipLaunchKernelGGL(k_lv_lists, dim3(nbt), dim3(256), 0, st, segs, ns, key, na, tile_cnt, posL, posR, segbase, (const uint32_t *) nullptr, (const uint32_t *) tile_seg);
          hipLaunchKernelGGL(k_lv_swap, dim3(nbt), dim3(256), 0, st, segs, ns, key, idx, na, segbase, posL, posR, (const uint32_t *) nullptr, (const uint32_t *) tile_seg);
        }
        hipLaunchKernelGGL(k_se_child_count, dim3(cdiv(ns, 256)), dim3(256), 0, st, segs, ns, cnt);
        prims::exclusive_scan<unsigned long long>(cnt, cnt, ns, b.scan_tmp, st);
        if (2ull * ns > max_segs) throw bk_error(BK_ERR_LIMIT, "std_sort_groups: segment list overflow");
        hipLaunchKernelGGL(k_se_child_write, dim3(cdiv(ns, 256)), dim3(256), 0, st, segs, ns, cnt, segs2, fin_list, fin, tile_seg);
        HIP_CHECK(hipMemcpyAsync(&tot, cnt + ns, 8, hipMemcpyDeviceToHost, st));
        HIP_CHECK(hipStreamSynchronize(st));
        std::swap(segs, segs2);
        ++level;
      }
      else
      {
        if (std::min<uint64_t>((uint64_t) ns << batch, (uint64_t) na / FIN_MAX + 1) > max_segs) throw bk_error(BK_ERR_LIMIT, "std_sort_groups: segment list overflow");
        const uint32_t cur[2] = {ns, na};
        if (level > 0) HIP_CHECK(hipMemcpyAsync(lvl, cur, 8, hipMemcpyHostToDevice, st));
        if (!pivoted) hipLaunchKernelGGL(k_se_pivot, dim3(cdiv(ns, 256)), dim3(256), 0, st, segs, ns, key, idx, err, heap_list);
        const unsigned nbt = cdiv(na, LV_TILE);
        uint32_t ns_bound = ns;
        for (int l = 0; l < batch; ++l)
        {
          {
            hipLaunchKernelGGL(k_lv_count, dim3(nbt), dim3(256), 0, st, segs, ns_bound, key, na, tile_cnt, (const uint32_t *) lvl, (const uint32_t *) tile_seg);
            hipLaunchKernelGGL(k_lv_sums, dim3(1), dim3(LV_SUM_THREADS), 0, st, tile_cnt, ns_bound, na, segbase, (const uint32_t *) lvl);
            hipLaunchKernelGGL(k_lv_lists, dim3(nbt), dim3(256), 0, st, segs, ns_bound, key, na, tile_cnt, posL, posR, segbase, (const uint32_t *) lvl, (const uint32_t *) tile_seg);
            hipLaunchKernelGGL(k_lv_swap, dim3(nbt), dim3(256), 0, st, segs, ns_bound, key, idx, na, segbase, posL, posR, (const uint32_t *) lvl, (const uint32_t *) tile_seg);
          }
          hipLaunchKernelGGL(k_se_children_small, dim3(1), dim3(CHILD_THREADS), 0, st, segs, lvl, segs2, fin_list, fin, key, idx, err, heap_list, tile_seg);
          std::swap(segs, segs2);
          ns_bound = ns_bound * 2 < CHILD_FUSED ? ns_bound * 2 : CHILD_FUSED;
          ++level;
        }
        pivoted = true;
        uint32_t now[3] = {0, 0, 0};
        HIP_CHECK(hipMemcpyAsync(now, lvl, 12, hipMemcpyDeviceToHost, st));
        HIP_CHECK(hipStreamSynchronize(st));
        tot = (unsigned long long) now[0] | ((unsigned long long) now[1] << 32);
        max_live = now[2];
      }
      const uint32_t ns2 = (uint32_t) tot;
      if (dbg_levels && (level % 4 == 0 || ns2 == 0))
      {
        HIP_CHECK(hipStreamSynchronize(st));
        fprintf(stderr, "[sortemu]   level %d: %u segments -> %u (%u live elements, largest %u), %.3f ms so far\n", level, ns, ns2, (uint32_t) (tot >> 32), max_live, now_ms() - t_loop0);
      }
      ns = ns2;
      na = (uint32_t) (tot >> 32);
      if (level > 200) throw bk_error(BK_ERR_LIMIT, "std_sort_groups: runaway recursion");
    }
  }
  if (chk) sort_check("after the partition levels", key, idx, key0, n, goff, ng, st, b);
  uint32_t hstate[ST_WORDS] = {};
  HIP_CHECK(hipMemcpyAsync(hstate, state, sizeof hstate, hipMemcpyDeviceToHost, st));
  HIP_CHECK(hipStreamSynchronize(st));
  uint32_t nfin2[2] = {hstate[ST_FIN], hstate[ST_FIN + 1]};
  uint32_t e[8];
  for (int k = 0; k < 8; ++k) e[k] = hstate[ST_ERR + k];
  if (e[0] & 8u) throw bk_error(BK_ERR_HIP, "std_sort_groups: k_se_tail_round lost a segment (list overflow or a cut outside its segment)");
  const uint32_t nfin = nfin2[0] + nfin2[1];
  const uint32_t nh1 = e[3], max1 = e[1], n_big = e[4];
  const HeapSeg *hl = reinterpret_cast<const HeapSeg *>(heap_list);
  static const bool dbg = bk_debug("sort");
  hent *hscratch = nullptr;
  uint32_t *scratch32 = nullptr, *scratch32b = nullptr;
  unsigned long long *rka = nullptr, *rkb = nullptr;
  hipEvent_t ev0 = nullptr, ev1 = nullptr;
  if (dbg)
  {
    HIP_CHECK(hipEventCreate(&ev0));
    HIP_CHECK(hipEventCreate(&ev1));
    HIP_CHECK(hipEventRecord(ev0, st));
  }
  if (nh1 || nfin) hscratch = b.heap_scratch.as<hent>((uint64_t) n + HEAP_PAD);
  if (b.heavy && nh1 && (max1 > HEAP_RANKED_MIN || b.heavy_all))
  {
// ... 118 lines not shown
```

breakid_amd/csrc/sortsvc.inc:

```

constexpr uint32_t SVC_T_PART = 1, SVC_T_FIN = 2, SVC_T_HEAP = 3;
constexpr uint32_t SVC_WIDE_MIN = 16384;
constexpr uint32_t SVC_BIAS = 0x80000000u;
constexpr uint32_t SVC_MAX_JOBS = 64;
constexpr uint32_t SVC_H_QUIT = 0, SVC_H_ERROR = 1, SVC_H_NARROW = 8, SVC_H_STARTED = 16, SVC_H_DONE = SVC_H_STARTED + 1024, SVC_H_WORDS = SVC_H_DONE + SVC_MAX_JOBS;
constexpr uint32_t SVC_NARROW_LDS = 45056;
constexpr unsigned long long SVC_TIMEOUT_TICKS = 800000000ull;

struct SvcTask
{
  uint32_t type_job;
  uint32_t first, last;
  int32_t depth;
};
static_assert(sizeof(SvcTask) == 16, "two 8-byte halves");

struct SvcJob
{
  uint32_t *key, *idx, *posL, *posR;
  hent *hscratch;
  uint32_t *scratch32, *scratch32b;
  unsigned long long *rka, *rkb;
  uint32_t remaining;
  uint32_t done;
  uint32_t max_heap;
  uint32_t n_heap;
  uint32_t epoch;
  uint32_t pad[3];
  unsigned long long t_submit, t_parts, t_done, last_heap;
};
static_assert(sizeof(SvcJob) % 8 == 0, "copied in 8-byte words");

struct SvcQueue
{
  uint32_t *head, *tail;
  SvcTask *slots;
  uint32_t *seq;
  uint32_t mask;
  uint32_t release;
};
struct SvcParams
{
  SvcQueue q[2];
  SvcJob *jobs;
  uint32_t *error;
  uint32_t *quit_d;
  uint32_t *host;
  uint32_t *stats;
  uint32_t cap32;
  uint32_t quit_word;
  unsigned long long timeout_ticks;
  uint32_t *pos[2];
  uint32_t pos_cap[2];
  uint32_t *dbg;
};

#define SVC_FAIL(P, code, a, b, c)                                  \
  do                                                                \
  {                                                                 \
    if (atomicOr((P).error, (code)) == 0u)                          \
    {                                                               \
      (P).error[8] = (code);                                        \
      (P).error[9] = (a);                                           \
      (P).error[10] = (b);                                          \
      (P).error[11] = (c);                                          \
    }                                                               \
  } while (0)
#define SVC_LD(p) __hip_atomic_load((p), __ATOMIC_RELAXED, __HIP_MEMORY_SCOPE_AGENT)
__device__ __forceinline__ uint32_t svc_read(uint32_t *p) { return atomicAdd(p, 0u); }
__device__ __forceinline__ unsigned long long svc_read(unsigned long long *p) { return atomicAdd(p, 0ull); }
__device__ __forceinline__ void svc_write(uint32_t *p, uint32_t v) { (void) atomicExch(p, v); }
__device__ __forceinline__ void svc_write(unsigned long long *p, unsigned long long v) { (void) atomicExch(p, v); }
#define SVC_ST(p, v) __hip_atomic_store((p), (v), __ATOMIC_RELAXED, __HIP_MEMORY_SCOPE_AGENT)
__device__ __forceinline__ void svc_release()
{
  __builtin_amdgcn_fence(__ATOMIC_RELEASE, "agent");
  asm volatile("s_waitcnt vmcnt(0)" ::: "memory");
}
__device__ __forceinline__ void svc_acquire()
{
  __builtin_amdgcn_fence(__ATOMIC_ACQUIRE, "agent");
  asm volatile("s_waitcnt vmcnt(0)" ::: "memory");
}

__device__ __forceinline__ void svc_drain_barrier()
{
  asm volatile("s_waitcnt vmcnt(0)" ::: "memory");
  __syncthreads();
}

__device__ __forceinline__ void svc_push(const SvcQueue &q, const SvcTask t, uint32_t *error)
{
  const uint32_t pos = atomicAdd(q.tail, 1u);
  const uint32_t slot = pos & q.mask;
  for (uint32_t spins = 0; svc_read(q.seq + slot) != pos; ++spins)
  {
    __builtin_amdgcn_s_sleep(16);
    if (spins > (1u << 22) || svc_read(error) != 0)
    {
      atomicOr(error, 2u);
      return;
    }
  }
  unsigned long long *d = reinterpret_cast<unsigned long long *>(q.slots + slot);
  svc_write(d, (unsigned long long) t.type_job | ((unsigned long long) t.first << 32));
  svc_write(d + 1, (unsigned long long) t.last | ((unsigned long long) (uint32_t) t.depth << 32));
  asm volatile("s_waitcnt vmcnt(0)" ::: "memory");
  svc_write(q.seq + slot, pos + 1u);
}
__device__ __forceinline__ uint32_t svc_ticket(const SvcQueue &q) { return atomicAdd(q.head, 1u); }
__device__ __forceinline__ bool svc_take(const SvcQueue &q, const uint32_t pos, SvcTask &t)
{
  const uint32_t slot = pos & q.mask;
  if (svc_read(q.seq + slot) != pos + 1u) return false;
  unsigned long long *s = reinterpret_cast<unsigned long long *>(q.slots + slot);
  const unsigned long long a = svc_read(s), b = svc_read(s + 1);
  t.type_job = (uint32_t) a;
  t.first = (uint32_t) (a >> 32);
  t.last = (uint32_t) b;
  t.depth = (int32_t) (uint32_t) (b >> 32);
  svc_write(q.seq + slot, pos + q.mask + 1u);
  return true;
}

__device__ __forceinline__ uint32_t svc_tag(uint32_t type, uint32_t job_tag) { return type | (job_tag << 4); }
__device__ __forceinline__ void svc_push_part(const SvcParams &P, uint32_t job_tag, uint32_t first, uint32_t last, int32_t depth)
{
  svc_push(P.q[(last - first) > SVC_WIDE_MIN ? 0 : 1], SvcTask{svc_tag(SVC_T_PART, job_tag), first, last, depth}, P.error);
}
__device__ __forceinline__ void svc_push_heap(const SvcParams &P, SvcJob *job, uint32_t job_tag, uint32_t first, uint32_t last)
{
  atomicMax(&job->max_heap, last - first);
  atomicAdd(&job->n_heap, last - first);
  svc_push(P.q[(last - first) > HEAP_BIG_MIN ? 0 : 1], SvcTask{svc_tag(SVC_T_HEAP, job_tag), first, last, 0}, P.error);
}
__device__ __forceinline__ void svc_done(const SvcParams &P, SvcJob *job, const uint32_t epoch)
{
  if (P.dbg) job->t_done = wall_clock64();
  svc_write(&job->done, 1u);
  __hip_atomic_store(P.host + SVC_H_DONE + (uint32_t) (job - P.jobs), epoch, __ATOMIC_RELAXED, __HIP_MEMORY_SCOPE_SYSTEM);
}
__device__ __forceinline__ void svc_retire(const SvcParams &P, SvcJob *job, const uint32_t job_tag, uint32_t dec)
{
  if (dec == 0) return;
  if (P.q[0].release & 2u) svc_release();
  if (atomicSub(&job->remaining, dec) == dec) svc_done(P, job, job_tag >> 8);
}

struct SvcJobLds
{
  uint32_t *key, *idx, *posL, *posR;
  hent *hscratch;
  uint32_t *scratch32, *scratch32b;
  unsigned long long *rka, *rkb;
  SvcJob *job;
  uint32_t tag;
};

__device__ __forceinline__ uint32_t svc_pick_pivot(uint32_t first, uint32_t last, uint32_t *key, uint32_t *idx)
{
  const uint32_t a = first + 1, b = first + (last - first) / 2, c = last - 1;
  const uint32_t ka = key[a], kb = key[b], kc = key[c];
  uint32_t pick;
  if (ka < kb)
  {
    if (kb < kc) pick = b;
    else if (ka < kc) pick = c;
    else pick = a;
  }
  else if (ka < kc) pick = a;
  else if (kb < kc) pick = c;
  else pick = b;
  const uint32_t kf = key[first], kp = key[pick];
  const uint32_t xf = idx[first], xp = idx[pick];
  st_through(key + first, kp);
  st_through(key + pick, kf);
  st_through(idx + first, xp);
  st_through(idx + pick, xf);
  return kp;
}

template <uint32_t NT> struct SvcPartLds
{
  uint32_t first, last, pivot;
  int32_t depth;
  uint32_t cnt[2][NT / 64];
  uint32_t cut;
  int go_on;
};
template <uint32_t NT, bool WIDE> __device__ __forceinline__ void svc_part(const SvcParams &P, const SvcJobLds &J, SvcPartLds<NT> &S, const SvcTask t, uint32_t *pos, const uint32_t pos_cap)
{
  constexpr uint32_t NW = NT / 64;
  const uint32_t tid = threadIdx.x, lane = tid & 63, w = tid >> 6;
  uint32_t *key = J.key, *idx = J.idx;
  const uint32_t job_tag = t.type_job >> 4;
  uint32_t retired = 0;
  if (tid == 0)
  {
    S.first = t.first;
    S.last = t.last;
    S.go_on = 1;
    if (t.depth == 0)
    {
      svc_push_heap(P, J.job, job_tag, t.first, t.last);
      S.go_on = 0;
    }
    else if (t.last - t.first > pos_cap + 1u)
    {
      atomicOr(P.error, 32u);
      S.go_on = 0;
    }
    else
    {
      S.pivot = svc_pick_pivot(t.first, t.last, key, idx);
      S.depth = t.depth - 1;
      S.cut = 0xFFFFFFFFu;
    }
  }
  __syncthreads();
  if (!S.go_on) return;
  unsigned long long tph = 0;
  uint32_t *phase = (P.dbg && WIDE) ? P.dbg + 12 * 8192 + 32 : nullptr;
  auto mark = [&](int k) {
    if (phase && tid == 0)
    {
      const unsigned long long now = wall_clock64();
      if (k >= 0) atomicAdd(phase + k, (uint32_t) (now - tph));
      tph = now;
    }
  };
  for (;;)
  {
    const uint32_t first = S.first, last = S.last, pivot = S.pivot;
    const int32_t depth = S.depth;
    mark(-1);
    if (phase && tid == 0) atomicAdd(phase + 7, 1u);
    const uint32_t lo = first + 1, total = last - lo;
    const uint32_t chunk = (((total + NW - 1) / NW) + 63u) & ~63u;
    const uint32_t wbeg = lo + min(total, w * chunk), wend = lo + min(total, (w + 1) * chunk);
    uint32_t cL = 0, cR = 0;
    {
      uint32_t p = wbeg + lane;
      for (; p + (TL_UNROLL - 1) * 64 < wend; p += TL_UNROLL * 64)
      {
        uint32_t k[TL_UNROLL];
#pragma unroll
        for (uint32_t u = 0; u < TL_UNROLL; ++u) k[u] = key[p + u * 64];
#pragma unroll
        for (uint32_t u = 0; u < TL_UNROLL; ++u)
        {
          cL += k[u] >= pivot ? 1u : 0u;
          cR += k[u] <= pivot ? 1u : 0u;
        }
      }
      for (; p < wend; p += 64)
      {
        const uint32_t k = key[p];
        cL += k >= pivot ? 1u : 0u;
        cR += k <= pivot ? 1u : 0u;
      }
    }
    for (int d = 32; d >= 1; d >>= 1)
    {
      cL += __shfl_xor(cL, d, 64);
      cR += __shfl_xor(cR, d, 64);
    }
    if (lane == 0)
    {
      S.cnt[0][w] = cL;
      S.cnt[1][w] = cR;
    }
    __syncthreads();
    mark(0);
    uint32_t runL = 0, runR = 0, nL = 0, nR = 0;
    for (uint32_t i = 0; i < NW; ++i)
    {
      const uint32_t a = S.cnt[0][i], b = S.cnt[1][i];
      if (i < w)
      {
        runL += a;
        runR += b;
      }
      nL += a;
      nR += b;
    }
    uint32_t *pL = pos, *pR = pos + pos_cap;
    {
      auto place = [&](uint32_t p, bool valid, uint32_t k) {
        const bool fL = valid && k >= pivot, fR = valid && k <= pivot;
        const unsigned long long mL = __ballot(fL), mR = __ballot(fR);
        const uint32_t bL = __builtin_amdgcn_mbcnt_hi((uint32_t) (mL >> 32), __builtin_amdgcn_mbcnt_lo((uint32_t) mL, 0u));
        const uint32_t bR = __builtin_amdgcn_mbcnt_hi((uint32_t) (mR >> 32), __builtin_amdgcn_mbcnt_lo((uint32_t) mR, 0u));
        if (fL) pL[runL + bL] = p;
        if (fR) pR[runR + bR] = p;
        runL += (uint32_t) __popcll(mL);
        runR += (uint32_t) __popcll(mR);
      };
      uint32_t p0 = wbeg;
      for (; p0 + TL_UNROLL * 64 <= wend; p0 += TL_UNROLL * 64)
      {
        uint32_t k[TL_UNROLL];
#pragma unroll
        for (uint32_t u = 0; u < TL_UNROLL; ++u) k[u] = key[p0 + u * 64 + lane];
#pragma unroll
        for (uint32_t u = 0; u < TL_UNROLL; ++u) place(p0 + u * 64 + lane, true, k[u]);
      }
      for (; p0 < wend; p0 += 64)
      {
        const uint32_t p = p0 + lane;
        const bool valid = p < wend;
        place(p, valid, valid ? key[p] : 0u);
      }
    }
    __syncthreads();
    mark(1);
    const uint32_t mm = nL < nR ? nL : nR;
    constexpr uint32_t SW = 4;
    for (uint32_t j0 = tid; j0 <= mm; j0 += SW * NT)
    {
      uint32_t lj[SW], rj[SW];
      bool sw[SW];
#pragma unroll
      for (uint32_t u = 0; u < SW; ++u)
      {
        const uint32_t j = j0 + u * NT;
        lj[u] = j < nL ? pL[j] : 0xFFFFFFFFu;
        rj[u] = j < nR ? pR[nR - 1 - j] : first;
      }
      uint32_t k1[SW], k2[SW], x1[SW], x2[SW];
#pragma unroll
      for (uint32_t u = 0; u < SW; ++u)
      {
        const uint32_t j = j0 + u * NT;
        sw[u] = j <= mm && (j < nL) && (j < nR) && (lj[u] < rj[u]);
        if (sw[u])
        {
          k1[u] = key[lj[u]];
          k2[u] = key[rj[u]];
          x1[u] = idx[lj[u]];
          x2[u] = idx[rj[u]];
        }
      }
#pragma unroll
      for (uint32_t u = 0; u < SW; ++u)
        if (sw[u])
        {
          st_through(key + lj[u], k2[u]);
          st_through(key + rj[u], k1[u]);
          st_through(idx + lj[u], x2[u]);
          st_through(idx + rj[u], x1[u]);
        }
#pragma unroll
      for (uint32_t u = 0; u < SW; ++u)
      {
        const uint32_t j = j0 + u * NT;
        if (j > mm || sw[u]) continue;
        const uint32_t ljj = lj[u];
        bool prev_cont = false;
        uint32_t rprev = 0;
        if (j > 0)
        {
          const uint32_t lp = pL[j - 1];
          rprev = pR[nR - j];
          prev_cont = lp < rprev;
        }
        if (j == 0)
          S.cut = ljj;
        else if (prev_cont)
          S.cut = ljj < rprev ? ljj : rprev;
      }
      if (!sw[SW - 1]) break;
    }
    svc_drain_barrier();
    mark(2);
    const uint32_t cut = S.cut;
    __syncthreads();
    if (cut == 0xFFFFFFFFu || cut <= first || cut > last)
    {
      if (tid == 0) SVC_FAIL(P, 8u, first, last, cut);
      return;
    }
    if (tid == 0)
    {
      const uint32_t a0 = first, a1 = cut, b0 = cut, b1 = last;
      const uint32_t sa = a1 - a0, sb = b1 - b0;
      const bool big_is_a = sa >= sb;
      const uint32_t g0 = big_is_a ? a0 : b0, g1 = big_is_a ? a1 : b1, h0 = big_is_a ? b0 : a0, h1 = big_is_a ? b1 : a1;
      const uint32_t sg = g1 - g0, sh = h1 - h0;
      const bool carry = sg > FIN_MAX && (!WIDE || sg > SVC_WIDE_MIN);
      const bool push_g = sg > 16 && !carry, push_h = sh > 16;
      retired += (sg <= 16 ? sg : 0u) + (sh <= 16 ? sh : 0u);
      const bool carry_heap = carry && depth == 0;
      if (push_g || push_h || carry_heap)
      {
        if (P.q[0].release & 1u) svc_release();
        if (push_h)
        {
          if (sh <= FIN_MAX)
            svc_push(P.q[1], SvcTask{svc_tag(SVC_T_FIN, job_tag), h0, h1, depth}, P.error);
          else
            svc_push_part(P, job_tag, h0, h1, depth);
        }
        if (push_g)
        {
          if (sg <= FIN_MAX)
            svc_push(P.q[1], SvcTask{svc_tag(SVC_T_FIN, job_tag), g0, g1, depth}, P.error);
          else
            svc_push_part(P, job_tag, g0, g1, depth);
        }
        if (carry_heap) svc_push_heap(P, J.job, job_tag, g0, g1);
      }
      if (carry && !carry_heap)
      {
        S.first = g0;
        S.last = g1;
        S.pivot = svc_pick_pivot(g0, g1, key, idx);
        S.depth = depth - 1;
        S.cut = 0xFFFFFFFFu;
        S.go_on = 1;
      }
      else
        S.go_on = 0;
    }
    svc_drain_barrier();
    mark(3);
    if (!S.go_on) break;
  }
  if (tid == 0 && retired) svc_retire(P, J.job, job_tag, retired);
}

constexpr uint32_t F2_HB = 256;
constexpr uint32_t F2_QCAP = 256;
constexpr uint32_t F2_EXT = 16;
struct Fin2Lds
{
  hent ent[FIN_MAX];
  uint16_t posL[FIN_MAX + 2], posR[FIN_MAX + 2];
  unsigned long long q[F2_QCAP];
  hent hbuf[4][F2_HB + 4];
  uint2 ext[F2_EXT];
  uint32_t q_head, q_tail, pending, n_ext, ext_elems, bad;
};
static_assert(sizeof(Fin2Lds) <= SVC_NARROW_LDS, "narrow workgroup LDS");
static_assert(FIN_MAX / F2_HB + 1 <= F2_EXT && FIN_MAX / 17 + 8 <= F2_QCAP, "fin2 lists");

__device__ __forceinline__ void f2_wsync()
{
  __builtin_amdgcn_fence(__ATOMIC_ACQ_REL, "wavefront");
  __builtin_amdgcn_wave_barrier();
}
__device__ __forceinline__ void f2_push(Fin2Lds &L, uint32_t first, uint32_t last, int32_t depth)
{
  const uint32_t slot = atomicAdd(&L.q_tail, 1u);
  if (slot >= F2_QCAP)
  {
    L.bad = 1u;
    return;
  }
  __hip_atomic_store(&L.q[slot], (unsigned long long) first | ((unsigned long long) last << 16) | ((unsigned long long) (uint32_t) (depth + 1) << 32), __ATOMIC_RELEASE, __HIP_MEMORY_SCOPE_WORKGROUP);
}
__device__ __forceinline__ uint32_t f2_partition(Fin2Lds &L, const uint32_t first, const uint32_t last, const uint32_t lane)
{
  hent *ent = L.ent;
  const uint32_t a = first + 1, b = first + (last - first) / 2, c = last - 1;
  const hent ea = ent[a], eb = ent[b], ec = ent[c];
  const uint32_t ka = hkey(ea), kb = hkey(eb), kc = hkey(ec);
  uint32_t pick;
  if (ka < kb)
  {
    if (kb < kc) pick = b;
    else if (ka < kc) pick = c;
    else pick = a;
  }
  else if (ka < kc) pick = a;
  else if (kb < kc) pick = c;
  else pick = b;
  const hent ep = pick == a ? ea : (pick == b ? eb : ec), ef = ent[first];
  const uint32_t pivot = hkey(ep);
  f2_wsync();
  if (lane == 0)
  {
    ent[first] = ep;
    ent[pick] = ef;
  }
  f2_wsync();
  uint16_t *pL = L.posL + first + 1, *pR = L.posR + first + 1;
  uint32_t nL = 0, nR = 0;
  for (uint32_t p0 = first + 1; p0 < last; p0 += 64)
  {
    const uint32_t p = p0 + lane;
    const bool valid = p < last;
    const uint32_t k = valid ? hkey(ent[p]) : 0u;
    const bool fL = valid && k >= pivot, fR = valid && k <= pivot;
    const unsigned long long mL = __ballot(fL), mR = __ballot(fR);
    if (fL) pL[nL + __builtin_amdgcn_mbcnt_hi((uint32_t) (mL >> 32), __builtin_amdgcn_mbcnt_lo((uint32_t) mL, 0u))] = (uint16_t) p;
    if (fR) pR[nR + __builtin_amdgcn_mbcnt_hi((uint32_t) (mR >> 32), __builtin_amdgcn_mbcnt_lo((uint32_t) mR, 0u))] = (uint16_t) p;
    nL += (uint32_t) __popcll(mL);
    nR += (uint32_t) __popcll(mR);
  }
  f2_wsync();
  const uint32_t mm = nL < nR ? nL : nR;
  uint32_t cut = 0xFFFFFFFFu;
  for (uint32_t j0 = 0; j0 <= mm; j0 += 64)
  {
    const uint32_t j = j0 + lane;
    const bool act = j <= mm;
    const uint32_t lj = act && j < nL ? pL[j] : 0xFFFFFFFFu;
    const uint32_t rj = act && j < nR ? pR[nR - 1 - j] : first;
    const bool sw = act && j < nL && j < nR && lj < rj;
    uint32_t mycut = 0xFFFFFFFFu;
    if (sw)
    {
      const hent e1 = ent[lj], e2 = ent[rj];
      ent[lj] = e2;
      ent[rj] = e1;
    }
    else if (act)
    {
      if (j == 0)
        mycut = lj;
      else
      {
        const uint32_t lp = pL[j - 1], rprev = pR[nR - j];
        if (lp < rprev) mycut = lj < rprev ? lj : rprev;
      }
    }
    const unsigned long long mc = __ballot(mycut != 0xFFFFFFFFu);
    if (mc != 0ull)
    {
      cut = __shfl(mycut, (int) __builtin_ctzll(mc), 64);
      break;
    }
  }
  f2_wsync();
  return cut;
}
__device__ __forceinline__ void fin2_body(Fin2Lds &L, const uint32_t g0, const uint32_t g1, const int32_t depth0, uint32_t *key, uint32_t *idx)
{
  const uint32_t tid = threadIdx.x, lane = tid & 63, w = tid >> 6, m = g1 - g0;
  for (uint32_t e = tid; e < m; e += 256) L.ent[e] = ((hent) key[g0 + e] << 32) | idx[g0 + e];
  for (uint32_t e = tid; e < F2_QCAP; e += 256) L.q[e] = 0ull;
  if (tid == 0)
  {
    L.q[0] = (unsigned long long) 0u | ((unsigned long long) m << 16) | ((unsigned long long) (uint32_t) (depth0 + 1) << 32);
    L.q_tail = 1;
    L.q_head = 0;
    L.pending = m;
    L.n_ext = 0;
    L.ext_elems = 0;
    L.bad = 0;
  }
  __syncthreads();
  for (;;)
  {
    uint32_t t = 0;
    if (lane == 0) t = atomicAdd(&L.q_head, 1u);
    t = __shfl(t, 0, 64);
    unsigned long long e = 0ull;
    bool done = false;
    for (;;)
    {
      if (t < F2_QCAP) e = __hip_atomic_load(&L.q[t], __ATOMIC_ACQUIRE, __HIP_MEMORY_SCOPE_WORKGROUP);
      if (e != 0ull) break;
      if (__hip_atomic_load(&L.pending, __ATOMIC_RELAXED, __HIP_MEMORY_SCOPE_WORKGROUP) == 0u || __hip_atomic_load(&L.bad, __ATOMIC_RELAXED, __HIP_MEMORY_SCOPE_WORKGROUP) != 0u)
      {
        done = true;
        break;
      }
      __builtin_amdgcn_s_sleep(2);
    }
    if (done) break;
    uint32_t first = (uint32_t) e & 0xFFFFu, last = (uint32_t) (e >> 16) & 0xFFFFu;
    int32_t depth = (int32_t) (uint32_t) (e >> 32) - 1;
    f2_wsync();
    for (;;)
    {
      const uint32_t sz = last - first;
      uint32_t retired = 0;
      bool go_on = false;
      if (depth == 0)
      {
        if (sz <= F2_HB)
        {
          hent *hb = L.hbuf[w];
          for (uint32_t i = lane; i < sz; i += 64) hb[i] = L.ent[first + i];
          f2_wsync();
          LdsMem mem{hb};
          make_heap_wave(mem, sz);
          sort_heap_asm<false>(hb, sz, 1);
          f2_wsync();
          for (uint32_t i = lane; i < sz; i += 64) L.ent[first + i] = hb[i];
          f2_wsync();
        }
        else if (lane == 0)
        {
          const uint32_t k = atomicAdd(&L.n_ext, 1u);
          if (k < F2_EXT) L.ext[k] = make_uint2(g0 + first, g0 + last); else L.bad = 1u;
          atomicAdd(&L.ext_elems, sz);
        }
        retired = sz;
      }
      else
      {
        const uint32_t cut = f2_partition(L, first, last, lane);
        if (cut <= first || cut > last)
        {
          if (lane == 0) L.bad = 2u;
          retired = sz;
        }
        else
        {
          const uint32_t sa = cut - first, sb = last - cut;
          const bool big_a = sa >= sb;
          const uint32_t h0 = big_a ? first : cut, h1 = big_a ? cut : last, l0 = big_a ? cut : first, l1 = big_a ? last : cut;
          const uint32_t sh = h1 - h0, sl = l1 - l0;
          --depth;
          if (sl > 16)
          {
            if (lane == 0) f2_push(L, l0, l1, depth);
          }
          else
            retired += sl;
          if (sh > 16)
          {
            first = h0;
            last = h1;
            go_on = true;
          }
          else
            retired += sh;
        }
      }
      if (retired && lane == 0) atomicSub(&L.pending, retired);
      if (!go_on) break;
    }
  }
  __syncthreads();
  for (uint32_t e = tid; e < m; e += 256)
  {
    const hent v = L.ent[e];
    st_through(key + g0 + e, hkey(v));
    st_through(idx + g0 + e, (uint32_t) v);
  }
}

static_assert((HEAP_BIG_MIN + HEAP_PAD) * 8 <= SVC_NARROW_LDS, "narrow workgroup LDS");

template <bool WIDE> __global__ __launch_bounds__(WIDE ? 1024 : 256) void k_sort_service(const SvcParams P)
{
  constexpr uint32_t NT = WIDE ? 1024u : 256u;
  extern __shared__ __attribute__((aligned(16))) unsigned char pool[];
  __shared__ SvcTask s_task;
  __shared__ int s_state;
  __shared__ SvcJobLds s_job;
  __shared__ SvcPartLds<NT> s_part;
  const uint32_t tid = threadIdx.x;
  const SvcQueue q = P.q[WIDE ? 0 : 1];
  if (tid == 0)
  {
    s_job.tag = 0xFFFFFFFFu;
    atomicAdd(P.stats + (WIDE ? 2 : 3), 1u);
    if (!WIDE && blockIdx.x == 0) __hip_atomic_store(P.host + SVC_H_NARROW, 1u, __ATOMIC_RELAXED, __HIP_MEMORY_SCOPE_SYSTEM);
    if (WIDE) __hip_atomic_store(P.host + SVC_H_STARTED + blockIdx.x, 1u, __ATOMIC_RELAXED, __HIP_MEMORY_SCOPE_SYSTEM);
  }
  unsigned long long t_last = wall_clock64();
  const unsigned long long t_start = t_last;
  uint32_t acc[8] = {0, 0, 0, 0, 0, 0, 0, 0};
  unsigned long long t_poll = t_last, t_task = t_last;
  for (;;)
  {
    if (tid == 0)
    {
      int st = 0;
      t_poll = wall_clock64();
      SvcTask t;
      uint32_t nap = 1, polls = 0;
      const uint32_t ticket = svc_ticket(q);
      uint32_t *dbg = P.dbg ? P.dbg + 4 * (blockIdx.x + (WIDE ? 0u : 4096u)) : nullptr;
      for (;;)
      {
        if (dbg)
        {
          SVC_ST(dbg, 1u);
          SVC_ST(dbg + 1, polls);
          SVC_ST(dbg + 2, (uint32_t) (wall_clock64() - t_start));
        }
        if (svc_take(q, ticket, t))
        {
          st = 1;
          break;
        }
        if (const uint32_t err = ((polls & 7u) == 0 ? svc_read(P.error) : 0u))
        {
          for (uint32_t k = 0; k < 4; ++k) __hip_atomic_store(P.host + SVC_H_ERROR + 1 + k, SVC_LD(P.error + 8 + k), __ATOMIC_RELAXED, __HIP_MEMORY_SCOPE_SYSTEM);
          __hip_atomic_store(P.host + SVC_H_ERROR, err, __ATOMIC_RELAXED, __HIP_MEMORY_SCOPE_SYSTEM);
          st = 2;
          if (dbg) SVC_ST(dbg + 3, 6u);
          break;
        }
        if ((++polls & 15u) == 0)
        {
          const uint32_t qv = svc_read(P.quit_d);
          if (qv == P.quit_word)
          {
            st = 2;
            if (dbg) SVC_ST(dbg + 3, 7u);
            break;
          }
          if (qv != 0u) atomicAdd(P.stats + 6, 1u);
        }
        if ((polls & 15u) == 0 && wall_clock64() - t_last > P.timeout_ticks)
        {
          atomicAdd(P.stats + (WIDE ? 4 : 5), 1u);
          st = 2;
          if (dbg) SVC_ST(dbg + 3, 8u);
          break;
        }
        for (uint32_t k = 0; k < nap; ++k) __builtin_amdgcn_s_sleep(32);
        if (nap < 4) ++nap;
      }
      if (st == 1)
      {
        svc_acquire();
        const uint32_t tag = t.type_job >> 4;
        if (s_job.tag != tag)
        {
          SvcJob *job = P.jobs + (tag & 0xFFu);
          unsigned long long *src = reinterpret_cast<unsigned long long *>(job);
          unsigned long long v[9];
#pragma unroll
          for (int k = 0; k < 9; ++k) v[k] = svc_read(src + k);
          s_job.key = (uint32_t *) v[0];
          s_job.idx = (uint32_t *) v[1];
          s_job.posL = (uint32_t *) v[2];
          s_job.posR = (uint32_t *) v[3];
          s_job.hscratch = (hent *) v[4];
          s_job.scratch32 = (uint32_t *) v[5];
          s_job.scratch32b = (uint32_t *) v[6];
          s_job.rka = (unsigned long long *) v[7];
          s_job.rkb = (unsigned long long *) v[8];
          s_job.job = job;
          s_job.tag = tag;
        }
        s_task = t;
      }
      s_state = st;
      if (dbg) SVC_ST(dbg, st == 1 ? 5u : 9u);
      t_task = wall_clock64();
      acc[0] += (uint32_t) (t_task - t_poll);
      if (dbg && st != 1)
      {
        uint32_t *a = P.dbg + 4 * 8192 + 8 * (blockIdx.x + (WIDE ? 0u : 4096u));
        for (int k = 0; k < 8; ++k) SVC_ST(a + k, acc[k]);
      }
    }
    __syncthreads();
    if (s_state != 1) return;
    const SvcTask t = s_task;
    const uint32_t type = t.type_job & 15u;
    if (P.dbg && tid == 0 && !WIDE && type != SVC_T_PART)
      atomicAdd(P.dbg + 12 * 8192 + (type == SVC_T_HEAP ? 16 : 0) + (31 - __clz((int) (t.last - t.first))), 1u);
    if (type == SVC_T_PART)
      svc_part<NT, WIDE>(P, s_job, s_part, t, P.pos[WIDE ? 0 : 1] + 2ull * P.pos_cap[WIDE ? 0 : 1] * blockIdx.x, P.pos_cap[WIDE ? 0 : 1]);
    else if (type == SVC_T_HEAP)
    {
      if (WIDE)
        heap_big_body(t.first, t.last, s_job.key, s_job.idx, s_job.hscratch, s_job.scratch32, s_job.scratch32b, s_job.rka, s_job.rkb, reinterpret_cast<hent *>(pool), P.cap32, NT);
      else
        heap_small_body(t.first, t.last, s_job.key, s_job.idx, reinterpret_cast<hent *>(pool), NT);
      svc_drain_barrier();
      if (tid == 0) svc_retire(P, s_job.job, t.type_job >> 4, t.last - t.first);
    }
    else if (type == SVC_T_FIN && !WIDE)
    {
      Fin2Lds &L = *reinterpret_cast<Fin2Lds *>(pool);
      fin2_body(L, t.first, t.last, t.depth, s_job.key, s_job.idx);
      svc_drain_barrier();
      if (tid == 0)
      {
        if (L.bad) SVC_FAIL(P, 64u, t.first, t.last, L.bad | (L.q_tail << 8) | (L.n_ext << 20));
        const uint32_t nh = L.n_ext < F2_EXT ? L.n_ext : F2_EXT;
        if (nh && (P.q[0].release & 1u)) svc_release();
        for (uint32_t k = 0; k < nh; ++k) svc_push_heap(P, s_job.job, t.type_job >> 4, L.ext[k].x, L.ext[k].y);
        svc_retire(P, s_job.job, t.type_job >> 4, (t.last - t.first) - L.ext_elems);
      }
    }
    else if (tid == 0)
      atomicOr(P.error, 16u);
    if (tid == 0)
    {
      t_last = wall_clock64();
      atomicAdd(P.stats + (WIDE ? 0 : 1), 1u);
      if (P.dbg)
      {
        if (type == SVC_T_HEAP)
          s_job.job->last_heap = ((unsigned long long) (t_last - t_task) << 32) | (t.last - t.first);
        else
          atomicMax(&s_job.job->t_parts, t_last);
      }
      const uint32_t dt = (uint32_t) (t_last - t_task), ty = type <= 3u ? type : 3u;
      acc[ty] += dt;
      acc[3 + ty] += 1u;
      acc[7] = dt > acc[7] ? dt : acc[7];
    }
    __syncthreads();
  }
}

__global__ __launch_bounds__(256) void k_svc_reset(const SvcParams P)
{
  const uint32_t i = blockIdx.x * blockDim.x + threadIdx.x;
  for (int k = 0; k < 2; ++k)
    if (i <= P.q[k].mask) P.q[k].seq[i] = i;
  if (i == 0)
  {
    for (int k = 0; k < 2; ++k) *P.q[k].head = *P.q[k].tail = 0u;
    *P.error = 0u;
    *P.quit_d = 0u;
    for (int k = 0; k < 8; ++k) P.stats[k] = 0u;
  }
  if (i < SVC_MAX_JOBS)
  {
    P.jobs[i].done = 0u;
    P.jobs[i].remaining = 0u;
  }
}

__global__ void k_svc_quit(uint32_t *quit_d, uint32_t word) { atomicExch(quit_d, word); }

__global__ __launch_bounds__(256) void k_svc_submit(const SvcParams P, const SvcJob desc, uint32_t slot, const uint64_t *__restrict__ goff, uint32_t ng)
{
  __shared__ uint32_t s_total;
  SvcJob *job = P.jobs + slot;
  const uint32_t job_tag = slot | (desc.epoch << 8);
  if (threadIdx.x == 0)
  {
    s_total = 0;
    const unsigned long long *src = reinterpret_cast<const unsigned long long *>(&desc);
    unsigned long long *dst = reinterpret_cast<unsigned long long *>(job);
    for (uint32_t k = 0; k < sizeof(SvcJob) / 8; ++k)
      if (k != 9) svc_write(dst + k, src[k]);
    svc_write(&job->done, 0u);
    svc_write(&job->remaining, SVC_BIAS);
    job->t_submit = wall_clock64();
    job->t_parts = 0ull;
    job->last_heap = 0ull;
    asm volatile("s_waitcnt vmcnt(0)" ::: "memory");
    svc_release();
  }
  __syncthreads();
  uint32_t mine = 0;
  for (uint32_t g = threadIdx.x; g < ng; g += blockDim.x)
  {
    const uint32_t first = (uint32_t) goff[g], last = (uint32_t) goff[g + 1], sz = last - first;
    if (sz <= 16) continue;
    mine += sz;
    const int32_t depth = 2 * (31 - __clz((int) sz));
    if (sz <= FIN_MAX)
      svc_push(P.q[1], SvcTask{svc_tag(SVC_T_FIN, job_tag), first, last, depth}, P.error);
    else
      svc_push_part(P, job_tag, first, last, depth);
  }
  atomicAdd(&s_total, mine);
  __syncthreads();
  if (threadIdx.x == 0)
  {
    const uint32_t add = s_total - SVC_BIAS;
    if (atomicAdd(&job->remaining, add) + add == 0u) svc_done(P, job, desc.epoch);
  }
}
```

include/breakid_hip.h:

```cpp
#ifndef BREAKID_HIP_H
#define BREAKID_HIP_H

#include <stdint.h>
#include <stddef.h>

#ifdef __cplusplus
extern "C" {
#endif

#define BK_OK 0
#define BK_ERR_ARG (-1)
#define BK_ERR_HIP (-2)
#define BK_ERR_NO_DEVICE (-3)
#define BK_ERR_UNSORTED (-4)
#define BK_ERR_CIGAR (-5)
#define BK_ERR_IO (-6)
#define BK_ERR_LIMIT (-7)
#define BK_ERR_COLLISION (-8)

#define BK_MEM_HOST 0
#define BK_MEM_DEVICE 1

typedef struct bk_ctx bk_ctx;

typedef struct bk_soa {
  uint64_t n;
  const int32_t *tid, *pos, *mtid, *mpos, *isize;
  const uint16_t *flag;
  const uint8_t *mapq;
  const uint64_t *qhash;
  const uint32_t *cigar_off;
  const uint32_t *cigar;
  const uint32_t *aux_off;
  const uint8_t *aux;
  uint64_t n_cigar_words;
  uint64_t n_aux_bytes;
  const uint32_t *qcheck;
  const struct bk_side *side;
} bk_soa;

typedef struct bk_side {
  uint64_t qhash;
  int32_t mtid, mpos;
  uint32_t qcheck;
  uint32_t reserved[3];
} bk_side;

typedef struct bk_pair {
  uint32_t x, y;
  uint32_t p1_pos, p2_pos;
  int32_t p1_tid, p2_tid;
  uint16_t p1_flag, p2_flag;
  uint8_t p1_mapq, p2_mapq, p1_rev, p2_rev;
  uint64_t rec;
  uint32_t id;
  int32_t cluster;
  uint32_t group;
  uint32_t reserved;
} bk_pair;

typedef struct bk_split {
  uint64_t rec;
  int32_t tid, pos, endpos;
  uint32_t reserved;
  uint64_t qhash;
  int32_t prim_chr, sec_chr;
  uint32_t prim_start, prim_end, prim_bp, sec_start, sec_end, sec_bp;
  uint64_t prim_cigar, sec_cigar;
  uint32_t flags;
  uint32_t qcheck;
} bk_split;

#define BK_TYPE_DIFF_CHR 1u
#define BK_TYPE_SAME_ORIENT 2u
#define BK_TYPE_ABS_REVERSE 4u
#define BK_TYPE_DEFAULT_ORIENT 8u

typedef struct bk_cluster {
  uint32_t group;
  int32_t id;
  int32_t p1_tid, p2_tid;
  uint32_t p1_mean, p2_mean, p1_min, p1_max, p2_min, p2_max;
  uint32_t p1_exact;
  int32_t p2_exact;
  uint32_t n_drp, n_sr;
  uint32_t depth1, depth2;
  uint32_t type_mask;
  uint32_t flags;
} bk_cluster;

#define BK_STAGE_SCAN 0
#define BK_STAGE_ISO 1
#define BK_STAGE_CLUSTERED 2
#define BK_STAGE_SPLITS 3
#define BK_STAGE_CLUSTERS 4
#define BK_STAGE_GROUP_KEYS 5

int bk_init(int device, const uint32_t *target_len, const char *const *target_name, int n_targets, bk_ctx **out);
void bk_prepare_process(void);
void bk_free(bk_ctx *ctx);
const char *bk_last_error(const bk_ctx *ctx);
int bk_set_stream(bk_ctx *ctx, void *hip_stream);
int bk_sync(bk_ctx *ctx);
int bk_get_stream(bk_ctx *ctx, void **hip_stream);

int bk_upload_records(bk_ctx *ctx, const bk_soa *cols, int mem_space);

int bk_isize_stats(bk_ctx *ctx, double *mean, double *sd);
int bk_discordant_pairs(bk_ctx *ctx, int mapq_min, double w, uint64_t *n_pairs, uint32_t *n_groups);
int bk_mask_and_cluster(bk_ctx *ctx, double w, int fast, uint64_t *n_clustered);
int bk_split_evidence(bk_ctx *ctx, uint64_t *n_tuples);
int bk_cluster_summary(bk_ctx *ctx, double w, uint64_t *n_clusters);
int bk_split_breakpoints(bk_ctx *ctx, double w, uint64_t *n_valid);

int bk_run(bk_ctx *ctx, int mapq_min, int fast, double *w_out, uint64_t *n_valid);

int bk_fetch(bk_ctx *ctx, int stage, const void **data, uint64_t *count, const uint64_t **group_off, uint32_t *n_groups);

typedef struct bk_group_stat {
  int32_t p1_tid, p2_tid;
  uint64_t n_scan, n_isolated_removed, n_clustered;
  uint32_t cluster_id_end;
  uint32_t ordinal;
} bk_group_stat;
int bk_group_stats(bk_ctx *ctx, const bk_group_stat **out, uint32_t *n_groups);

int bk_timing(bk_ctx *ctx, const char *const **names, const float **ms, const uint64_t **bytes, int *n);
int bk_timing_enable(bk_ctx *ctx, int on);
int bk_timing_touched(bk_ctx *ctx, const uint64_t **touched, int *n);

typedef struct bk_shard_stats {
  uint64_t isize_sum, isize_n;
  double sumsq;
  uint32_t vmax, max_span;
  uint64_t n_cand, n_split;
} bk_shard_stats;
#define BK_BUF_CANDIDATES 0
#define BK_BUF_TUPLES 1
#define BK_BUF_CLUSTERS 2
int bk_shard_begin(bk_ctx *ctx, uint64_t rec_base, int mapq_min);
int bk_shard_get_stats(bk_ctx *ctx, bk_shard_stats *out);
int bk_shard_set_stats(bk_ctx *ctx, const bk_shard_stats *total);
int bk_shard_sd_local(bk_ctx *ctx, uint64_t *l_total, void **ex_dev, uint64_t *n_ex);
int bk_shard_sd_finish(bk_ctx *ctx, const void *all_ex_dev, uint64_t n_all, uint64_t l_grand, double *mean, double *sd);
int bk_shard_buffer(bk_ctx *ctx, int which, void **dev, uint64_t *count, uint32_t *elem_bytes);
int bk_shard_set_buffer(bk_ctx *ctx, int which, const void *dev, uint64_t count);
int bk_shard_group_sizes(bk_ctx *ctx, const uint64_t **starts, uint32_t *n_groups);
int bk_shard_own_groups(bk_ctx *ctx, const uint8_t *own, uint32_t n_groups);
int bk_shard_route_candidates(bk_ctx *ctx, uint32_t world, void **dev, const uint64_t **counts);
int bk_shard_group_keys(bk_ctx *ctx, const uint32_t **keys, uint32_t *n_groups);
int bk_shard_route_pairs(bk_ctx *ctx, const uint32_t *dest_of_group, uint32_t n_groups, uint32_t world, void **dev, const uint64_t **counts);
int bk_shard_group_pairs(bk_ctx *ctx, const void *pairs_dev, uint64_t n, const uint32_t *all_keys, uint32_t n_all_keys);
int bk_shard_bp_cov(bk_ctx *ctx, double w, void **cov_dev, uint64_t *n);
int bk_shard_bp_vote(bk_ctx *ctx, double w, const void *cov_total_dev);
int bk_shard_bp_vote_slice(bk_ctx *ctx, double w, const void *cov_total_dev, uint64_t lo, uint64_t hi, void **clusters_dev, void **voted_dev);
int bk_shard_bp_set_voted(bk_ctx *ctx, const void *voted_all_dev);
int bk_shard_bp_depth(bk_ctx *ctx, void **depth_dev, uint64_t *n);
int bk_shard_bp_finish(bk_ctx *ctx, const void *depth_total_dev);

int bk_debug_std_sort(bk_ctx *ctx, const uint32_t *key, const uint64_t *group_off, uint32_t n_groups, uint32_t *perm_out);

int bk_debug_ahc(bk_ctx *ctx, const uint32_t *x, const uint32_t *y, uint32_t n, double w, uint32_t *idx_out, int32_t *cluster_out, uint32_t *n_out);

int bk_debug_points(bk_ctx *ctx, int mode, const uint32_t *x, const uint32_t *y, uint32_t n, double w, uint32_t *idx_out, int32_t *cluster_out, uint32_t *n_out);
int bk_debug_cigar(bk_ctx *ctx, uint32_t n, const uint8_t *kind, const uint32_t *c1_off, const uint8_t *c1, const uint32_t *c2_off, const uint8_t *c2, const int32_t *e,
                   int32_t *out6);
int bk_debug_vote(bk_ctx *ctx, const bk_split *side1, uint32_t n1, const bk_split *side2, uint32_t n2, int32_t p1_tid, int32_t p2_tid, int32_t *out3);
int bk_debug_region(bk_ctx *ctx, int32_t tid, uint32_t start, uint32_t end, uint64_t depth_pos, bk_split *out, uint32_t cap, uint32_t *n_out, uint32_t *cov_out,
                    uint32_t *depth_out);

typedef struct bk_bam bk_bam;
uint64_t bk_qname_hash(const char *name, size_t len);
uint32_t bk_qname_check(const char *name, size_t len);
int bk_bam_open(const char *path, bk_bam **out, char *err, size_t errlen);
int bk_bam_header(const bk_bam *b, int *n_targets, const char *const **names, const uint32_t **lens);
int bk_bam_decode(bk_bam *b, bk_soa *out, char *err, size_t errlen);
void bk_bam_close(bk_bam *b);

typedef struct bk_bam_dev bk_bam_dev;
int bk_bam_decode_device(const char *path, int device, bk_bam_dev **out, bk_soa *cols, int *n_targets, const char *const **names, const uint32_t **lens,
                         char *err, size_t errlen);
int bk_bam_decode_device_part(const char *path, int device, int part, int parts, bk_bam_dev **out, bk_soa *cols, int *n_targets, const char *const **names,
                              const uint32_t **lens, char *err, size_t errlen);
void bk_bam_dev_free(bk_bam_dev *h);
void bk_feed_release_caches(void);
int bk_bam_decode_device_ctx(const char *path, int device, int mapq_min, bk_bam_dev **bam_out, bk_ctx **ctx_out, int *n_targets, const char *const **names,
                             const uint32_t **lens, char *err, size_t errlen);
int bk_debug_bgzf_inflate(const void *file, uint64_t n, void *out, uint64_t out_cap, uint64_t *out_len, float *kernel_ms, char *err, size_t errlen);

#ifdef __cplusplus
}
#endif
#endif
```

Measured before the change: 10330.

## Run per-stream group sorts as a one-shot task-queue dispatch kernel

When the persistent sort service is not running, grouped sorts are now executed by a single launched kernel whose workgroups pull partition, heap and finisher tasks from device queues. Wide workgroups handle big partitions and heaps, while narrow workgroups split into four 256-thread teams with LDS-based team barriers. This replaces the multi-kernel fin-list/segment path and its many launches. It adds a blocking host read of group offsets and a sync for error checking, plus a timeout and an env switch to fall back. A counter API reports which sort form ran.

```diff
diff --git a/breakid_amd/capi.py b/breakid_amd/capi.py
--- a/breakid_amd/capi.py
+++ b/breakid_amd/capi.py
@@ -30,7 +30,7 @@
 EXPORTS = ["bk_init", "bk_prepare_process", "bk_free", "bk_last_error", "bk_set_stream", "bk_sync", "bk_get_stream", "bk_upload_records", "bk_isize_stats",
            "bk_discordant_pairs", "bk_mask_and_cluster", "bk_split_evidence", "bk_cluster_summary",
            "bk_split_breakpoints", "bk_run", "bk_fetch", "bk_timing", "bk_timing_enable", "bk_timing_touched", "bk_group_stats", "bk_qname_hash", "bk_qname_check",
-           "bk_bam_open", "bk_bam_header", "bk_bam_decode", "bk_bam_close", "bk_bam_decode_device", "bk_bam_decode_device_part", "bk_bam_decode_device_ctx", "bk_bam_dev_free", "bk_feed_release_caches", "bk_debug_bgzf_inflate", "bk_debug_std_sort", "bk_debug_ahc", "bk_debug_points", "bk_debug_cigar", "bk_debug_vote", "bk_debug_region", "bk_shard_begin", "bk_shard_get_stats", "bk_shard_set_stats",
+           "bk_bam_open", "bk_bam_header", "bk_bam_decode", "bk_bam_close", "bk_bam_decode_device", "bk_bam_decode_device_part", "bk_bam_decode_device_ctx", "bk_bam_dev_free", "bk_feed_release_caches", "bk_debug_bgzf_inflate", "bk_debug_std_sort", "bk_sort_forms", "bk_debug_ahc", "bk_debug_points", "bk_debug_cigar", "bk_debug_vote", "bk_debug_region", "bk_shard_begin", "bk_shard_get_stats", "bk_shard_set_stats",
            "bk_shard_sd_local", "bk_shard_sd_finish", "bk_shard_buffer", "bk_shard_set_buffer", "bk_shard_group_sizes",
            "bk_shard_own_groups", "bk_shard_route_candidates", "bk_shard_group_keys", "bk_shard_route_pairs", "bk_shard_group_pairs", "bk_shard_bp_cov", "bk_shard_bp_vote", "bk_shard_bp_vote_slice", "bk_shard_bp_set_voted", "bk_shard_bp_depth", "bk_shard_bp_finish"]
 
@@ -67,6 +67,7 @@
         L.bk_timing_enable.argtypes = [vp, C.c_int]
         L.bk_timing_touched.argtypes = [vp, C.POINTER(C.POINTER(C.c_uint64)), C.POINTER(C.c_int)]
         L.bk_debug_std_sort.argtypes = [vp, vp, vp, C.c_uint32, vp]
+        L.bk_sort_forms.argtypes = [vp, u64p]
         L.bk_debug_ahc.argtypes = [vp, vp, vp, C.c_uint32, C.c_double, vp, vp, C.POINTER(C.c_uint32)]
         L.bk_debug_points.argtypes = [vp, C.c_int, vp, vp, C.c_uint32, C.c_double, vp, vp, C.POINTER(C.c_uint32)]
         L.bk_debug_cigar.argtypes = [vp, C.c_uint32, vp, vp, vp, vp, vp, vp, vp]
@@ -239,6 +240,11 @@
         self._check(self.L.bk_debug_std_sort(self.h, key.ctypes.data, group_off.ctypes.data, len(group_off) - 1, perm.ctypes.data))
         return perm
 
+    def sort_forms(self):
+        out = (C.c_uint64 * 3)()
+        self._check(self.L.bk_sort_forms(self.h, out))
+        return tuple(int(v) for v in out)
+
     def debug_ahc(self, x, y, w):
         x = np.ascontiguousarray(x, np.uint32)
         y = np.ascontiguousarray(y, np.uint32)
diff --git a/breakid_amd/csrc/api.hip b/breakid_amd/csrc/api.hip
--- a/breakid_amd/csrc/api.hip
+++ b/breakid_amd/csrc/api.hip
@@ -983,6 +983,7 @@
     ctx->cb.se.fork_heaps = fork;
     for (int k = 0; k < K - 1; ++k) ctx->lanes[k]->cb.se.fork_heaps = fork;
     if (!use_svc && bk_debug("lanes")) fprintf(stderr, "[lanes] launch path: %d lanes, %d stream%s each, %d hardware queues\n", K, fork ? 2 : 1, fork ? "s" : "", g_hw_queues_at_init);
+    if (!use_svc && sort_tasks_on() && bk_debug("lanes")) fprintf(stderr, "[lanes] sorts as task dispatches on the lane streams\n");
   }
   const bool adapt = !use_svc;
   auto lane_cb = [&](int l) -> ClusterBufs & { return l == 0 ? ctx->cb : ctx->lanes[l - 1]->cb; };
@@ -1583,6 +1584,18 @@
   });
 }
 
+int bk_sort_forms(bk_ctx *ctx, uint64_t out[3])
+{
+  return guarded(ctx, [&] {
+    if (!out) throw bk_error(BK_ERR_ARG, "bk_sort_forms: null output");
+    for (int k = 0; k < 3; ++k)
+    {
+      out[k] = ctx->cb.se.sorts[k];
+      for (const auto &l : ctx->lanes) out[k] += l->cb.se.sorts[k];
+    }
+  });
+}
+
 int bk_debug_ahc(bk_ctx *ctx, const uint32_t *x, const uint32_t *y, uint32_t n, double w, uint32_t *idx_out, int32_t *cluster_out, uint32_t *n_out)
 {
   return guarded(ctx, [&] {
diff --git a/breakid_amd/csrc/sortemu.h b/breakid_amd/csrc/sortemu.h
--- a/breakid_amd/csrc/sortemu.h
+++ b/breakid_amd/csrc/sortemu.h
@@ -37,6 +37,10 @@
   std::vector<uint32_t> *heavy = nullptr;
   bool heavy_all = false;
   bool fork_heaps = true;
+  DevBuf tj_ctl, tj_jobs, tj_slots[2], tj_seq[2], tj_pos[2], tj_heavy, tj_trace;
+  uint32_t tj_cap[2] = {0, 0}, tj_epoch = 0;
+  bool tj_ready = false;
+  uint64_t sorts[3] = {0, 0, 0};
   static constexpr int N_AUX = 5;
   hipStream_t aux[N_AUX] = {};
   hipEvent_t fork = nullptr, join[N_AUX] = {};
@@ -54,4 +58,6 @@
   }
 };
 
+bool sort_tasks_on();
+
 void std_sort_groups(uint32_t *key, uint32_t *idx, const uint32_t *gof, const uint64_t *goff, uint32_t ng, uint64_t n, SortEmuBufs &b, hipStream_t st);
diff --git a/breakid_amd/csrc/sortemu.hip b/breakid_amd/csrc/sortemu.hip
--- a/breakid_amd/csrc/sortemu.hip
+++ b/breakid_amd/csrc/sortemu.hip
@@ -1075,20 +1075,63 @@
     }
   }
 }
-__device__ __forceinline__ void heap_small_body(const uint32_t first, const uint32_t last, uint32_t *key, uint32_t *idx, hent *buf, const uint32_t NT)
-{
-  const uint32_t m = last - first;
+struct WgTeam
+{
+  __device__ __forceinline__ uint32_t tid() const { return threadIdx.x; }
+  __device__ __forceinline__ void sync() const { __syncthreads(); }
+  __device__ __forceinline__ void count_pushes(uint32_t) const {}
+};
+struct WgLive : WgTeam
+{
+  uint32_t *live;
+  __device__ __forceinline__ void count_pushes(uint32_t k) const
+  {
+    if (k) atomicAdd(live, k);
+  }
+};
+struct LdsTeam
+{
+  uint32_t *bar;
+  uint32_t base;
+  uint32_t *live;
+  __device__ __forceinline__ uint32_t tid() const { return threadIdx.x - base; }
+  __device__ __forceinline__ void sync() const
+  {
+    __builtin_amdgcn_fence(__ATOMIC_RELEASE, "workgroup");
+    if ((threadIdx.x & 63u) == 0)
+    {
+      const uint32_t g = __hip_atomic_load(bar + 1, __ATOMIC_RELAXED, __HIP_MEMORY_SCOPE_WORKGROUP);
+      if (__hip_atomic_fetch_add(bar, 1u, __ATOMIC_ACQ_REL, __HIP_MEMORY_SCOPE_WORKGROUP) == 3u)
+      {
+        __hip_atomic_store(bar, 0u, __ATOMIC_RELAXED, __HIP_MEMORY_SCOPE_WORKGROUP);
+        __hip_atomic_store(bar + 1, g + 1u, __ATOMIC_RELEASE, __HIP_MEMORY_SCOPE_WORKGROUP);
+      }
+      else
+        while (__hip_atomic_load(bar + 1, __ATOMIC_RELAXED, __HIP_MEMORY_SCOPE_WORKGROUP) == g) __builtin_amdgcn_s_sleep(1);
+    }
+    __builtin_amdgcn_wave_barrier();
+    __builtin_amdgcn_fence(__ATOMIC_ACQUIRE, "workgroup");
+  }
+  __device__ __forceinline__ void count_pushes(uint32_t k) const
+  {
+    if (k) atomicAdd(live, k);
+  }
+};
+
+template <class T = WgTeam> __device__ __forceinline__ void heap_small_body(const uint32_t first, const uint32_t last, uint32_t *key, uint32_t *idx, hent *buf, const uint32_t NT, const T &team = T())
+{
+  const uint32_t m = last - first, tid = team.tid();
   uint32_t *gk = key + first, *gx = idx + first;
-  for (uint32_t i = threadIdx.x; i < m; i += NT) buf[i] = ((hent) gk[i] << 32) | gx[i];
-  __syncthreads();
-  if (threadIdx.x < 64)
+  for (uint32_t i = tid; i < m; i += NT) buf[i] = ((hent) gk[i] << 32) | gx[i];
+  team.sync();
+  if (tid < 64)
   {
     LdsMem mem{buf};
     make_heap_wave(mem, m);
     sort_heap_asm<false>(buf, m, 1);
   }
-  __syncthreads();
-  for (uint32_t i = threadIdx.x; i < m; i += NT)
+  team.sync();
+  for (uint32_t i = tid; i < m; i += NT)
   {
     const hent e = buf[i];
     st_through(gk + i, hkey(e));
@@ -2498,6 +2541,140 @@
   window_sorts(key, idx, gof, n, st);
 }
 
+static void std_sort_groups_tasks(uint32_t *key, uint32_t *idx, const uint32_t *gof, const uint64_t *goff, uint32_t ng, uint32_t n, SortEmuBufs &b, hipStream_t st, const uint32_t *key0)
+{
+  static size_t dyn_lds = 0;
+  static uint32_t cap32 = 0;
+  static std::once_flag once;
+  std::call_once(once, [] {
+    hipFuncAttributes fa;
+    HIP_CHECK(hipFuncGetAttributes(&fa, reinterpret_cast<const void *>(k_sort_job)));
+    dyn_lds = (size_t) ((160u * 1024u - (uint32_t) fa.sharedSizeBytes) & ~15u);
+    cap32 = (uint32_t) (dyn_lds / 4 - 3);
+    if ((cap32 & 1u) == 0) --cap32;
+    if (dyn_lds < SJ_TEAMS * SJ_TEAM_LDS) throw bk_error(BK_ERR_HIP, "k_sort_job: the narrow teams do not fit the LDS");
+    HIP_CHECK(hipFuncSetAttribute(reinterpret_cast<const void *>(k_sort_job), hipFuncAttributeMaxDynamicSharedMemorySize, (int) dyn_lds));
+  });
+  std::vector<uint64_t> go((size_t) ng + 1);
+  HIP_CHECK(hipMemcpyAsync(go.data(), goff, go.size() * 8, hipMemcpyDeviceToHost, st));
+  HIP_CHECK(hipStreamSynchronize(st));
+  uint64_t max_group = 0;
+  for (uint32_t g = 0; g < ng; ++g) max_group = std::max<uint64_t>(max_group, go[g + 1] - go[g]);
+  const uint32_t n_wide = std::min<uint32_t>(SJ_MAX_WIDE, std::max<uint32_t>(1, cdiv(n, 1u << 16)));
+  const uint32_t n_narrow = std::min<uint32_t>(SJ_MAX_NARROW, std::max<uint32_t>(1, cdiv(n, 1u << 16)));
+  SjParams S = {};
+  SvcParams &P = S.P;
+  {
+    auto pow2 = [](uint64_t v) {
+      uint32_t c = 1024;
+      while (c < v && c < (1u << 30)) c <<= 1;
+      return c;
+    };
+    const uint32_t want[2] = {pow2((uint64_t) n / HEAP_BIG_MIN + 4096), pow2((uint64_t) n / 16 + 4096)};
+    for (int k = 0; k < 2; ++k)
+      if (want[k] > b.tj_cap[k])
+      {
+        b.tj_cap[k] = want[k];
+        b.tj_ready = false;
+      }
+    uint32_t *ctl = b.tj_ctl.as<uint32_t>(SJ_C_WORDS);
+    for (int k = 0; k < 2; ++k)
+    {
+      P.q[k].head = ctl + 64 * k;
+      P.q[k].tail = ctl + 64 * k + 32;
+      P.q[k].slots = b.tj_slots[k].as<SvcTask>(b.tj_cap[k]);
+      P.q[k].seq = b.tj_seq[k].as<uint32_t>(b.tj_cap[k]);
+      P.q[k].mask = b.tj_cap[k] - 1;
+      P.q[k].release = 1u;
+    }
+    P.error = ctl + SJ_C_ERROR;
+    P.stats = ctl + SJ_C_STATS;
+    P.quit_d = ctl + SJ_C_QUIT;
+    P.host = ctl + SJ_C_HOST;
+    P.jobs = b.tj_jobs.as<SvcJob>(SVC_MAX_JOBS);
+    P.cap32 = cap32;
+    P.quit_word = 0u;
+    P.timeout_ticks = SJ_TIMEOUT_TICKS;
+    P.pos_cap[0] = (uint32_t) std::max<uint64_t>(max_group, SVC_WIDE_MIN) + 64;
+    P.pos_cap[1] = SVC_WIDE_MIN + 64;
+    P.pos[0] = b.tj_pos[0].as<uint32_t>(2ull * P.pos_cap[0] * n_wide);
+    P.pos[1] = b.tj_pos[1].as<uint32_t>(2ull * P.pos_cap[1] * n_narrow * SJ_TEAMS);
+    P.dbg = nullptr;
+    S.n_wide = n_wide;
+    S.live = ctl + SJ_C_LIVE;
+    S.gof = gof;
+    S.heavy_min = b.heavy_all ? FIN_MAX : HEAP_RANKED_MIN;
+    if (b.heavy)
+    {
+      S.heavy = b.tj_heavy.as<uint32_t>(ng);
+      HIP_CHECK(hipMemsetAsync(S.heavy, 0, (size_t) ng * 4, st));
+    }
+  }
+  static const bool dbg = bk_debug("svc");
+  if (dbg) S.trace = b.tj_trace.as<unsigned long long>(8);
+  if (!b.tj_ready)
+  {
+    HIP_CHECK(hipMemsetAsync(b.tj_ctl.p, 0, SJ_C_WORDS * 4, st));
+    hipLaunchKernelGGL(k_svc_reset, dim3(cdiv(std::max(b.tj_cap[0], b.tj_cap[1]), 256)), dim3(256), 0, st, P);
+    b.tj_ready = true;
+  }
+  SvcJob d = {};
+  d.key = key;
+  d.idx = idx;
+  d.hscratch = b.heap_scratch.as<hent>((uint64_t) n + HEAP_PAD);
+  d.scratch32 = b.scratch32.as<uint32_t>((uint64_t) n + HEAP_PAD);
+  d.scratch32b = b.scratch32b.as<uint32_t>((uint64_t) n + HEAP_PAD);
+  d.rka = b.rk_a.as<unsigned long long>((uint64_t) n + HEAP_PAD);
+  d.rkb = b.rk_b.as<unsigned long long>((uint64_t) n + HEAP_PAD);
+  d.epoch = (b.tj_epoch++ % 0xFFFFFu) + 1u;
+  const SvcJobLds J = {d.key, d.idx, nullptr, nullptr, d.hscratch, d.scratch32, d.scratch32b, d.rka, d.rkb, P.jobs, d.epoch << 8};
+  hipLaunchKernelGGL(k_sort_job_submit, dim3(1), dim3(256), 0, st, S, d, goff, ng);
+  hipLaunchKernelGGL(k_sort_job, dim3(n_wide + n_narrow), dim3(1024), dyn_lds, st, S, J);
+  HIP_CHECK(hipGetLastError());
+  ++b.sorts[1];
+  if (key0) sort_check("after the task dispatch", key, idx, key0, n, goff, ng, st, b);
+  window_sorts(key, idx, gof, n, st);
+  uint32_t h[16] = {};
+  HIP_CHECK(hipMemcpyAsync(h, P.error, 12 * 4, hipMemcpyDeviceToHost, st));
+  std::vector<uint32_t> hv;
+  if (S.heavy)
+  {
+    hv.resize(ng);
+    HIP_CHECK(hipMemcpyAsync(hv.data(), S.heavy, (size_t) ng * 4, hipMemcpyDeviceToHost, st));
+  }
+  unsigned long long tr[8] = {};
+  if (S.trace) HIP_CHECK(hipMemcpyAsync(tr, S.trace, 5 * 8, hipMemcpyDeviceToHost, st));
+  SvcJob j = {};
+  HIP_CHECK(hipMemcpyAsync(&j, P.jobs, sizeof j, hipMemcpyDeviceToHost, st));
+  HIP_CHECK(hipStreamSynchronize(st));
+  if (h[0] || j.remaining != 0u)
+  {
+    b.tj_ready = false;
+    throw bk_error(h[0] & 2u ? BK_ERR_LIMIT : BK_ERR_HIP, "sort task dispatch: task error " + std::to_string(h[0]) + " (2 = ring overflow, 4 = no progress for 1 s, 8 = a cut outside its segment, 16 = a task in the wrong queue, 32 = a node beyond the position lists, 64 = the finisher), " + std::to_string(j.remaining) + " elements not final; first failing task: code " + std::to_string(h[8]) + ", " + std::to_string(h[9]) + " " + std::to_string(h[10]) + " " + std::to_string(h[11]));
+  }
+  if (S.heavy)
+  {
+    if (b.heavy->size() < ng) b.heavy->resize(ng, 0u);
+    for (uint32_t g = 0; g < ng; ++g) (*b.heavy)[g] = std::max((*b.heavy)[g], hv[g]);
+  }
+  if (S.trace)
+  {
+    const double t0 = (double) tr[0];
+    const uint32_t hm = (uint32_t) (tr[1] >> 40);
+    const unsigned long long hs = tr[1] & 0xFFFFFFFFFFull, base = tr[0] & ~0xFFFFFFFFFFull;
+    unsigned long long hstart = base | hs;
+    if (hstart < tr[0]) hstart += 1ull << 40;
+    fprintf(stderr, "[svc] task dispatch %u: %u elements in %u groups on %u wide + %u narrow workgroups; longest heap %u elements started %.3f ms after the dispatch and took %.3f ms; partitions and finisher done after %.3f ms, job after %.3f ms; %u elements in heaps, the longest %u\n",
+            d.epoch, n, ng, n_wide, n_narrow, hm, hm ? ((double) hstart - t0) * 1e-5 : 0.0, hm ? (double) (tr[2] & 0xFFFFFFFFFFull) * 1e-5 : 0.0, tr[3] ? ((double) tr[3] - t0) * 1e-5 : 0.0, ((double) tr[4] - t0) * 1e-5, j.n_heap, j.max_heap);
+  }
+}
+
+bool sort_tasks_on()
+{
+  static const bool on = !(getenv("BREAKID_SORT_TASKS") && atoi(getenv("BREAKID_SORT_TASKS")) == 0);
+  return on;
+}
+
 void std_sort_groups(uint32_t *key, uint32_t *idx, const uint32_t *gof, const uint64_t *goff, uint32_t ng, uint64_t n64, SortEmuBufs &b, hipStream_t st)
 {
   if (n64 == 0 || ng == 0) return;
@@ -2520,6 +2697,7 @@
   const uint32_t n = (uint32_t) n64;
   if (b.svc && b.svc->running)
   {
+    ++b.sorts[0];
     std_sort_groups_svc(key, idx, gof, goff, ng, n, b, st);
     return;
   }
@@ -2565,6 +2743,12 @@
     }
     ++call;
   }
+  if (sort_tasks_on())
+  {
+    std_sort_groups_tasks(key, idx, gof, goff, ng, n, b, st, chk ? key0 : nullptr);
+    return;
+  }
+  ++b.sorts[2];
   const uint32_t fin_cap = (uint32_t) ((uint64_t) n / 16 + ng + 16);
   FinSeg *fin_list = b.fin_list.as<FinSeg>(fin_cap);
   size_t max_segs = (size_t) n / 8 + ng + 16;
diff --git a/breakid_amd/csrc/sortsvc.inc b/breakid_amd/csrc/sortsvc.inc
--- a/breakid_amd/csrc/sortsvc.inc
+++ b/breakid_amd/csrc/sortsvc.inc
@@ -83,10 +83,10 @@
   asm volatile("s_waitcnt vmcnt(0)" ::: "memory");
 }
 
-__device__ __forceinline__ void svc_drain_barrier()
+template <class T = WgTeam> __device__ __forceinline__ void svc_drain_barrier(const T &team = T())
 {
   asm volatile("s_waitcnt vmcnt(0)" ::: "memory");
-  __syncthreads();
+  team.sync();
 }
 
 __device__ __forceinline__ void svc_push(const SvcQueue &q, const SvcTask t, uint32_t *error)
@@ -188,10 +188,11 @@
   uint32_t cut;
   int go_on;
 };
-template <uint32_t NT, bool WIDE> __device__ __forceinline__ void svc_part(const SvcParams &P, const SvcJobLds &J, SvcPartLds<NT> &S, const SvcTask t, uint32_t *pos, const uint32_t pos_cap)
+template <uint32_t NT, bool WIDE, class T = WgTeam>
+__device__ __forceinline__ void svc_part(const SvcParams &P, const SvcJobLds &J, SvcPartLds<NT> &S, const SvcTask t, uint32_t *pos, const uint32_t pos_cap, const T &team = T())
 {
   constexpr uint32_t NW = NT / 64;
-  const uint32_t tid = threadIdx.x, lane = tid & 63, w = tid >> 6;
+  const uint32_t tid = team.tid(), lane = tid & 63, w = tid >> 6;
   uint32_t *key = J.key, *idx = J.idx;
   const uint32_t job_tag = t.type_job >> 4;
   uint32_t retired = 0;
@@ -217,7 +218,7 @@
       S.cut = 0xFFFFFFFFu;
     }
   }
-  __syncthreads();
+  team.sync();
   if (!S.go_on) return;
   unsigned long long tph = 0;
   uint32_t *phase = (P.dbg && WIDE) ? P.dbg + 12 * 8192 + 32 : nullptr;
@@ -270,7 +271,7 @@
       S.cnt[0][w] = cL;
       S.cnt[1][w] = cR;
     }
-    __syncthreads();
+    team.sync();
     mark(0);
     uint32_t runL = 0, runR = 0, nL = 0, nR = 0;
     for (uint32_t i = 0; i < NW; ++i)
@@ -312,7 +313,7 @@
         place(p, valid, valid ? key[p] : 0u);
       }
     }
-    __syncthreads();
+    team.sync();
     mark(1);
     const uint32_t mm = nL < nR ? nL : nR;
     constexpr uint32_t SW = 4;
@@ -371,10 +372,10 @@
       }
       if (!sw[SW - 1]) break;
     }
-    svc_drain_barrier();
+    svc_drain_barrier(team);
     mark(2);
     const uint32_t cut = S.cut;
-    __syncthreads();
+    team.sync();
     if (cut == 0xFFFFFFFFu || cut <= first || cut > last)
     {
       if (tid == 0) SVC_FAIL(P, 8u, first, last, cut);
@@ -393,6 +394,7 @@
       const bool carry_heap = carry && depth == 0;
       if (push_g || push_h || carry_heap)
       {
+        team.count_pushes((push_h ? 1u : 0u) + (push_g ? 1u : 0u));
         if (P.q[0].release & 1u) svc_release();
         if (push_h)
         {
@@ -422,7 +424,7 @@
       else
         S.go_on = 0;
     }
-    svc_drain_barrier();
+    svc_drain_barrier(team);
     mark(3);
     if (!S.go_on) break;
   }
@@ -535,9 +537,9 @@
   f2_wsync();
   return cut;
 }
-__device__ __forceinline__ void fin2_body(Fin2Lds &L, const uint32_t g0, const uint32_t g1, const int32_t depth0, uint32_t *key, uint32_t *idx)
-{
-  const uint32_t tid = threadIdx.x, lane = tid & 63, w = tid >> 6, m = g1 - g0;
+template <class T = WgTeam> __device__ __forceinline__ void fin2_body(Fin2Lds &L, const uint32_t g0, const uint32_t g1, const int32_t depth0, uint32_t *key, uint32_t *idx, const T &team = T())
+{
+  const uint32_t tid = team.tid(), lane = tid & 63, w = tid >> 6, m = g1 - g0;
   for (uint32_t e = tid; e < m; e += 256) L.ent[e] = ((hent) key[g0 + e] << 32) | idx[g0 + e];
   for (uint32_t e = tid; e < F2_QCAP; e += 256) L.q[e] = 0ull;
   if (tid == 0)
@@ -550,7 +552,7 @@
     L.ext_elems = 0;
     L.bad = 0;
   }
-  __syncthreads();
+  team.sync();
   for (;;)
   {
     uint32_t t = 0;
@@ -635,7 +637,7 @@
       if (!go_on) break;
     }
   }
-  __syncthreads();
+  team.sync();
   for (uint32_t e = tid; e < m; e += 256)
   {
     const hent v = L.ent[e];
@@ -869,3 +871,215 @@
     if (atomicAdd(&job->remaining, add) + add == 0u) svc_done(P, job, desc.epoch);
   }
 }
+
+constexpr uint32_t SJ_TEAMS = 4;
+constexpr size_t SJ_TEAM_LDS = ((sizeof(Fin2Lds) > (HEAP_BIG_MIN + HEAP_PAD) * 8 ? sizeof(Fin2Lds) : (HEAP_BIG_MIN + HEAP_PAD) * 8) + 15) & ~(size_t) 15;
+static_assert(SJ_TEAMS * SJ_TEAM_LDS + 4096 <= 160 * 1024, "four narrow teams in a CU's LDS");
+constexpr uint32_t SJ_MAX_WIDE = 32, SJ_MAX_NARROW = 32;
+constexpr unsigned long long SJ_TIMEOUT_TICKS = 100000000ull;
+constexpr uint32_t SJ_C_ERROR = 128, SJ_C_STATS = 160, SJ_C_QUIT = 192, SJ_C_LIVE = 224, SJ_C_HOST = 256, SJ_C_WORDS = SJ_C_HOST + SVC_H_WORDS;
+
+struct SjParams
+{
+  SvcParams P;
+  uint32_t n_wide;
+  uint32_t *live;
+  uint32_t *heavy;
+  const uint32_t *gof;
+  uint32_t heavy_min;
+  unsigned long long *trace;
+};
+
+template <bool WIDE, class T>
+__device__ __forceinline__ void sj_serve(const SjParams &S, const SvcJobLds &J, SvcTask &s_task, int &s_state, SvcPartLds<WIDE ? 1024u : 256u> &s_part, unsigned char *pool, uint32_t *pos, const T &team)
+{
+  constexpr uint32_t NT = WIDE ? 1024u : 256u;
+  const SvcParams &P = S.P;
+  const SvcQueue &q = P.q[WIDE ? 0 : 1];
+  const uint32_t tid = team.tid();
+  SvcJob *job = J.job;
+  unsigned long long t_last = wall_clock64(), t_task = t_last;
+  if (S.trace && tid == 0) atomicMin(S.trace, t_last);
+  for (;;)
+  {
+    if (tid == 0)
+    {
+      int st = 0;
+      SvcTask t;
+      const uint32_t ticket = svc_ticket(q);
+      for (uint32_t polls = 0, nap = 1;; ++polls)
+      {
+        if (svc_take(q, ticket, t))
+        {
+          st = 1;
+          break;
+        }
+        if ((polls & 7u) == 0)
+        {
+          if (svc_read(P.error) != 0u || svc_read(&job->remaining) == 0u)
+          {
+            st = 2;
+            break;
+          }
+          if (svc_read(S.live) == 0u)
+          {
+            st = svc_take(q, ticket, t) ? 1 : 2;
+            break;
+          }
+          if (wall_clock64() - t_last > P.timeout_ticks)
+          {
+            SVC_FAIL(P, 4u, WIDE ? 1u : 0u, svc_read(&job->remaining), svc_read(S.live));
+            st = 2;
+            break;
+          }
+        }
+        for (uint32_t k = 0; k < nap; ++k) __builtin_amdgcn_s_sleep(32);
+        if (nap < 4) ++nap;
+      }
+      if (st == 1) svc_acquire();
+      s_task = t;
+      s_state = st;
+      t_task = wall_clock64();
+    }
+    team.sync();
+    if (s_state != 1) return;
+    const SvcTask t = s_task;
+    const uint32_t type = t.type_job & 15u, job_tag = t.type_job >> 4;
+    if (type == SVC_T_PART)
+    {
+      svc_part<NT, WIDE, T>(P, J, s_part, t, pos, P.pos_cap[WIDE ? 0 : 1], team);
+      if (tid == 0)
+      {
+        asm volatile("s_waitcnt vmcnt(0)" ::: "memory");
+        atomicSub(S.live, 1u);
+      }
+    }
+    else if (type == SVC_T_HEAP)
+    {
+      const uint32_t m = t.last - t.first;
+      if (WIDE)
+        heap_big_body(t.first, t.last, J.key, J.idx, J.hscratch, J.scratch32, J.scratch32b, J.rka, J.rkb, reinterpret_cast<hent *>(pool), P.cap32, NT);
+      else
+        heap_small_body<T>(t.first, t.last, J.key, J.idx, reinterpret_cast<hent *>(pool), NT, team);
+      svc_drain_barrier(team);
+      if (tid == 0)
+      {
+        if (S.heavy && m > S.heavy_min) atomicMax(S.heavy + S.gof[t.first], m);
+        if (S.trace)
+        {
+          const unsigned long long now = wall_clock64();
+          atomicMax(S.trace + 1, ((unsigned long long) m << 40) | (t_task & 0xFFFFFFFFFFull));
+          atomicMax(S.trace + 2, ((unsigned long long) m << 40) | ((now - t_task) & 0xFFFFFFFFFFull));
+        }
+        svc_retire(P, job, job_tag, m);
+      }
+    }
+    else if (type == SVC_T_FIN && !WIDE)
+    {
+      Fin2Lds &L = *reinterpret_cast<Fin2Lds *>(pool);
+      fin2_body<T>(L, t.first, t.last, t.depth, J.key, J.idx, team);
+      svc_drain_barrier(team);
+      if (tid == 0)
+      {
+        if (L.bad) SVC_FAIL(P, 64u, t.first, t.last, L.bad | (L.q_tail << 8) | (L.n_ext << 20));
+        const uint32_t nh = L.n_ext < F2_EXT ? L.n_ext : F2_EXT;
+        if (nh && (P.q[0].release & 1u)) svc_release();
+        for (uint32_t k = 0; k < nh; ++k) svc_push_heap(P, job, job_tag, L.ext[k].x, L.ext[k].y);
+        svc_retire(P, job, job_tag, (t.last - t.first) - L.ext_elems);
+        asm volatile("s_waitcnt vmcnt(0)" ::: "memory");
+        atomicSub(S.live, 1u);
+      }
+    }
+    else if (tid == 0)
+      SVC_FAIL(P, 16u, type, t.first, t.last);
+    if (tid == 0)
+    {
+      t_last = wall_clock64();
+      if (S.trace)
+      {
+        if (type != SVC_T_HEAP) atomicMax(S.trace + 3, t_last);
+        atomicMax(S.trace + 4, t_last);
+      }
+    }
+    team.sync();
+  }
+}
+
+__global__ __launch_bounds__(1024) void k_sort_job(const SjParams S, const SvcJobLds J)
+{
+  extern __shared__ __attribute__((aligned(16))) unsigned char pool[];
+  __shared__ SvcTask s_task[SJ_TEAMS];
+  __shared__ int s_state[SJ_TEAMS];
+  __shared__ uint32_t s_bar[SJ_TEAMS][2];
+  __shared__ union
+  {
+    SvcPartLds<1024> wide;
+    SvcPartLds<256> narrow[SJ_TEAMS];
+  } s_part;
+  if (blockIdx.x < S.n_wide)
+  {
+    sj_serve<true>(S, J, s_task[0], s_state[0], s_part.wide, pool, S.P.pos[0] + 2ull * S.P.pos_cap[0] * blockIdx.x, WgLive{{}, S.live});
+    return;
+  }
+  const uint32_t team = threadIdx.x >> 8;
+  if ((threadIdx.x & 255u) == 0)
+  {
+    s_bar[team][0] = 0u;
+    s_bar[team][1] = 0u;
+  }
+  __syncthreads();
+  sj_serve<false>(S, J, s_task[team], s_state[team], s_part.narrow[team], pool + team * SJ_TEAM_LDS,
+                  S.P.pos[1] + 2ull * S.P.pos_cap[1] * ((blockIdx.x - S.n_wide) * SJ_TEAMS + team), LdsTeam{s_bar[team], team * 256u, S.live});
+}
+
+__global__ __launch_bounds__(256) void k_sort_job_submit(const SjParams S, const SvcJob desc, const uint64_t *__restrict__ goff, uint32_t ng)
+{
+  __shared__ uint32_t s_total, s_tasks;
+  const SvcParams &P = S.P;
+  SvcJob *job = P.jobs;
+  const uint32_t job_tag = desc.epoch << 8;
+  if (threadIdx.x == 0)
+  {
+    s_total = 0;
+    s_tasks = 0;
+    for (int k = 0; k < 2; ++k) svc_write(P.q[k].head, svc_read(P.q[k].tail));
+    for (int k = 0; k < 12; ++k) svc_write(P.error + k, 0u);
+    svc_write(S.live, 0u);
+    if (S.trace)
+    {
+      svc_write(S.trace, ~0ull);
+      for (int k = 1; k < 5; ++k) svc_write(S.trace + k, 0ull);
+    }
+    const unsigned long long *src = reinterpret_cast<const unsigned long long *>(&desc);
+    unsigned long long *dst = reinterpret_cast<unsigned long long *>(job);
+    for (uint32_t k = 0; k < sizeof(SvcJob) / 8; ++k)
+      if (k != 9) svc_write(dst + k, src[k]);
+    svc_write(&job->done, 0u);
+    svc_write(&job->remaining, SVC_BIAS);
+    asm volatile("s_waitcnt vmcnt(0)" ::: "memory");
+    svc_release();
+  }
+  __syncthreads();
+  uint32_t mine = 0, tasks = 0;
+  for (uint32_t g = threadIdx.x; g < ng; g += blockDim.x)
+  {
+    const uint32_t first = (uint32_t) goff[g], last = (uint32_t) goff[g + 1], sz = last - first;
+    if (sz <= 16) continue;
+    mine += sz;
+    ++tasks;
+    const int32_t depth = 2 * (31 - __clz((int) sz));
+    if (sz <= FIN_MAX)
+      svc_push(P.q[1], SvcTask{svc_tag(SVC_T_FIN, job_tag), first, last, depth}, P.error);
+    else
+      svc_push_part(P, job_tag, first, last, depth);
+  }
+  atomicAdd(&s_total, mine);
+  atomicAdd(&s_tasks, tasks);
+  __syncthreads();
+  if (threadIdx.x == 0)
+  {
+    svc_write(S.live, s_tasks);
+    const uint32_t add = s_total - SVC_BIAS;
+    if (atomicAdd(&job->remaining, add) + add == 0u) svc_done(P, job, desc.epoch);
+  }
+}
diff --git a/include/breakid_hip.h b/include/breakid_hip.h
--- a/include/breakid_hip.h
+++ b/include/breakid_hip.h
@@ -160,6 +160,8 @@
 
 int bk_debug_std_sort(bk_ctx *ctx, const uint32_t *key, const uint64_t *group_off, uint32_t n_groups, uint32_t *perm_out);
 
+int bk_sort_forms(bk_ctx *ctx, uint64_t out[3]);
+
 int bk_debug_ahc(bk_ctx *ctx, const uint32_t *x, const uint32_t *y, uint32_t n, double w, uint32_t *idx_out, int32_t *cluster_out, uint32_t *n_out);
 
 int bk_debug_points(bk_ctx *ctx, int mode, const uint32_t *x, const uint32_t *y, uint32_t n, double w, uint32_t *idx_out, int32_t *cluster_out, uint32_t *n_out);
```

Measured after the change: 11760 (median of 6 runs). +13.9%, better.
